# UCL-CCS/symmer

Measured on AMD Instinct MI355X. Metric: pauli_term_pairs_per_sec, higher is better.
Workload: dtype u64

## Files before the change

include/symgpu.h:

```cpp
#ifndef SYMGPU_H
#define SYMGPU_H
#include <stdint.h>

#ifdef __cplusplus
extern "C" {
#endif

#define SYMGPU_OK 0
#define SYMGPU_E_INVALID (-1)
#define SYMGPU_E_HIP (-2)
#define SYMGPU_E_NOMEM (-3)
#define SYMGPU_E_CAPACITY (-4)
#define SYMGPU_E_NODEVICE (-5)
#define SYMGPU_E_COLLISION (-6)
#define SYMGPU_E_RCCL (-7)

typedef struct symgpu_op_s *symgpu_op_t;

#define SYMGPU_MAX_DEVICES 16
int symgpu_init(int device);
int symgpu_init_all(int n_devices);
int symgpu_set_device(int device);
int symgpu_current_device(int *device);
int symgpu_n_initialised(int *n);
int symgpu_shutdown(void);
const char *symgpu_last_error(void);
int symgpu_device_count(int *n);
int symgpu_sync(void);
int symgpu_device_sync(void);
int symgpu_device_name(char *buf, int len);
int symgpu_mem_info(int64_t *free_bytes, int64_t *total_bytes);
int symgpu_timer_start(void);
int symgpu_timer_stop(float *ms);
#define SYMGPU_PROF_CLASSES 6
int symgpu_prof_enable(int kernel_class, int on);
int symgpu_prof_read(int kernel_class, int64_t *n_launches, double *total_ms);
#define SYMGPU_COUNTER_LIST(X) \
    X(HASH_RESEEDS, 0, "number of row-hash collisions that forced the cleanup to reseed its hash and retry (the exactness guard behind " \
      "symplectic_cleanup, operators/utils.py:230-279; expected 0 outside the tests, which weaken the hash on purpose)") \
    X(RESIDENT_DONE, 1, "rotations completed by the one-launch LDS-resident kernel") \
    X(RESIDENT_FAILED, 2, "calls of that kernel that reported a failed row verification or a barrier time-out (the multi-launch path then " \
      "recomputes)") \
    X(DEV_MALLOC_CALLS, 3, "device allocations that were not served from the allocator's arena") \
    X(RESIDENT_NS_PREPARE, 4, "host nanoseconds spent by the one-launch rotation in preparation") \
    X(RESIDENT_NS_LAUNCH, 5, "host nanoseconds spent by the one-launch rotation in the launch call") \
    X(RESIDENT_NS_WAIT, 6, "host nanoseconds spent by the one-launch rotation waiting for the kernel's status word") \
     \
    X(H2D_BYTES, 7, "payload bytes copied host -> device by this library (operators, coefficients, index arrays, result matrices; not the " \
      "few-byte counts and flags a call reads back)") \
    X(D2H_BYTES, 8, "payload bytes copied device -> host by this library (as 7)") \
    X(OP_UPLOADS, 9, "operator uploads (calls that moved a whole operator or its coefficients)") \
    X(OP_DOWNLOADS, 10, "operator downloads (calls that moved a whole operator or its coefficients)") \
    X(CANARY_HITS, 11, "device blocks whose guard bytes were overwritten (tuning build, SYMGPU_ALLOC_CANARY)") \
    X(CTX_MAX_THREADS, 12, "the most threads seen using one device's context at once since load, counted where a call uses the context's " \
      "state, whichever lock it took (1 while the per-device lock holds)") \
    X(CTX_WAITS, 13, "calls that found their device busy with another thread's call and waited") \
    X(CTX_UNLOCKED_USES, 14, "uses of a device's context by a call that did not hold that context's lock (0 while the lock is taken on the " \
      "right device)") \
     \
    X(GF2_BLOCKS_PANELLED, 15, "blocks (of up to 64 rows) panelled by the blocked GF(2) elimination since load - the one-workgroup path for " \
      "matrices of at most 64 rows and 64 words counts none") \
    X(GF2_PANEL_FULL_ROWS, 16, "of 15, the blocks whose panel ran on the full rows in LDS") \
    X(GF2_PANEL_WINDOW, 17, "of 15, the blocks whose panel ran on the two-word window (the rest took the four-word window, or held zero " \
      "rows only)") \
     \
    X(COMMUTE_REGISTER_TILE, 18, "commutation calls (symgpu_commutes, symgpu_commutes_dev, symgpu_commutes_bits_dev and what is built on " \
      "them) served by the register-tile kernel") \
    X(COMMUTE_WIDE_ROWS, 19, "commutation calls served by the wide-row kernel") \
    X(COMMUTE_M4R_TILE, 20, "launches of the Four-Russians commutation kernel with one tile per workgroup (a stream-K request with fewer " \
      "tiles than compute units counts here)") \
    X(COMMUTE_M4R_STREAMK, 21, "launches of the Four-Russians commutation kernel as stream-K (persistent workgroups over the (tile, step) " \
      "space)") \
     \
    X(CHAIN_REGISTERS, 22, "runs of Clifford rotations (symgpu_rotate_clifford_chain_dev with at least one row and one rotation, and the " \
      "runs that symgpu_perform_rotations_dev hands to it) served by the register chain") \
    X(CHAIN_LDS, 23, "runs of Clifford rotations served by the LDS-resident kernel") \
    X(CHAIN_SINGLE_WORKGROUP, 24, "runs of Clifford rotations served by the single-workgroup kernel") \
    X(CHAIN_TWO_LAUNCHES, 25, "runs of Clifford rotations served by the two-launch form") \
    X(CHAIN_FOUR_LAUNCHES, 26, "runs of Clifford rotations served by the four-launch form") \
    X(CHAIN_SORT_ONE_LAUNCH, 27, "segments (of up to 40 rotations) of the register chain whose keys were sorted by the one-launch sort (a " \
      "run that is redone after a time-out of the one-launch sort counts 27 and 28)") \
    X(CHAIN_SORT_LAUNCHES, 28, "segments (of up to 40 rotations) of the register chain whose keys were sorted by the multi-launch sort") \
    X(ROTATE_HASH_JOIN, 29, "single rotations (symgpu_rotate_single_dev) completed by the hash join") \
    X(ROTATE_CLIFFORD_FAST, 30, "single rotations completed by the Clifford fast path") \
    X(ROTATE_GENERAL, 31, "single rotations completed by the general path (stack + cleanup)") \
    X(ROTATE_GENERAL_BY_DUP_CHECK, 32, "of 31, odd-k Clifford rotations whose duplicate check found two equal rows") \
     \
    X(RESIDENT_LDS, 33, "one-launch rotations LAUNCHED (completed or not) with each block's rows in LDS") \
    X(RESIDENT_REGISTERS, 34, "one-launch rotations LAUNCHED (completed or not) with each block's rows in LDS and registers") \
    X(RESIDENT_ROWS_IN_MEMORY, 35, "one-launch rotations LAUNCHED (completed or not) with each block's rows left in memory") \
     \
    X(FLOW_COMPLETE_SORT, 36, "the packed pair keys were ordered by the complete sort, no flag pass") \
    X(FLOW_FLAGS_HASH_TABLES, 37, "the flag pass was launched from the bucketed operand hash tables") \
    X(FLOW_FLAGS_PARTIAL_SORT, 38, "the flag pass was launched behind the partial sort") \
    X(FLOW_FLAGS_GAVE_UP, 39, "a flag pass came back with its give-up word set") \
    X(GIVEUP_PRODUCT_BUCKET, 40, "of 39, the hash-table pass by reason (one each for every reason it reported): a product bucket of more " \
      "than 16,384 pairs") \
    X(GIVEUP_COUNTER_SATURATED, 41, "of 39, the hash-table pass by reason: a saturated 4-bit counter") \
    X(GIVEUP_LIST_OVERFLOW, 42, "of 39, the hash-table pass by reason: an overflowing list") \
    X(GIVEUP_OPERAND_BUCKET, 43, "of 39, the hash-table pass by reason: an operand bucket of more than 255 terms") \
    X(FLOW_SORTED_WHOLE, 44, "the sort was finished on the whole array after the flag pass (most keys flagged, a give-up, or " \
      "SYMGPU_CLEANUP_SUSPECTS=2)") \
    X(FLOW_SORTED_FLAGGED, 45, "the flagged keys were sorted alone") \
    X(FLOW_MARKED_FROM_BYTES, 46, "the single terms were marked from one byte per pair") \
    X(FLOW_FULL_SORT_REPEAT, 47, "the attempt was repeated with the full 64-bit sort (a long run of equal key prefixes that holds " \
      "different keys)") \
     \
    X(PRODUCT_ROWS_ONLY, 48, "all-pairs products by path: rows only") \
    X(PRODUCT_PHASE_STREAM, 49, "all-pairs products by path: phase-byte row stream") \
    X(PRODUCT_WIDE_COEFF_THEN_ROWS, 50, "all-pairs products by path: wide coefficient kernel, then rows") \
    X(PRODUCT_WORD_MAJOR_THEN_ROWS, 51, "all-pairs products by path: word-major coefficient kernel, then rows") \
    X(PRODUCT_WORD_MAJOR_BESIDE_ROWS, 52, "all-pairs products by path: the same beside the rows on a second stream") \
     \
    X(CSR_FILL_LDS, 53, "launches of the fill kernel of symgpu_to_csr_fill (k_csr_fill) with its slots in LDS") \
    X(CSR_FILL_SCRATCH, 54, "launches of the fill kernel of symgpu_to_csr_fill (k_csr_fill) with its slots in global scratch") \
     \
    X(DEV_BLOCKS_LIVE, 55, "a GAUGE, not a count: device blocks handed out by the allocator and not yet returned to it (operators, their " \
      "caches, scratch, what the contexts keep); never below 0") \
    X(DEV_FREE_UNKNOWN, 56, "blocks returned to the allocator that it did not hold (a double free, a pointer from elsewhere); the call " \
      "fails with SYMGPU_E_INVALID and nothing is released") \
     \
    X(OP_WORD_MAJOR_BUILDS, 57, "word-major copies of an operator's rows built into its handle (op_wordmajor, layout.hip)") \
    X(OP_BIT_MAJOR_BUILDS, 58, "bit-major copies of an operator's rows built into its handle for the Four-Russians commutation kernel " \
      "(m4r_bit_major, commute_m4r.hip; a copy built into the call's scratch counts nothing)") \
    X(OP_YCOUNT_BUILDS, 59, "Y-count arrays built into an operator's handle (op_ycount, layout.hip)") \
    X(OP_ROW_HASH_BUILDS, 60, "row-hash arrays computed from an operand's rows into its handle (analyze_rows, rotate_analyze.hip; " \
      "ensure_row_hashes, rotate_resident.hip); hashes a rotation hands on to its result count nothing")
#define SYMGPU_COUNTER_ENUM_ENTRY(name, id, text) SYMGPU_CTR_##name = id,
typedef enum symgpu_counter { SYMGPU_COUNTER_LIST(SYMGPU_COUNTER_ENUM_ENTRY) SYMGPU_CTR_COUNT = 61 } symgpu_counter;
#undef SYMGPU_COUNTER_ENUM_ENTRY
int symgpu_debug_counter(int which, int64_t *value);
const char *symgpu_debug_counter_name(int which);
int symgpu_debug_sort(uint64_t *keys, uint32_t *vals, int64_t n, int begin_bit, int end_bit, int form, int with_first_hist, int *form_ran);
int symgpu_debug_scan(const uint32_t *in, uint32_t *out, int64_t n, uint32_t *total);
int symgpu_debug_popc_scan(const uint64_t *bits, int64_t n_words, int64_t n32, uint32_t *out, uint32_t *total);
int symgpu_degraded(char *buf, int len);
int symgpu_debug_rotation_trace(uint64_t *out, int max_workgroups, int *n_workgroups);

int symgpu_membw_probe(int64_t bytes, double *fill_GBps, double *copy_GBps);

int symgpu_op_upload(const uint64_t *rows, const double *coeff , int64_t T, int Wq, symgpu_op_t *out);
int symgpu_op_alloc(int64_t capacity_rows, int Wq, int with_coeff, symgpu_op_t *out);
int symgpu_op_download(symgpu_op_t op, uint64_t *rows, double *coeff , int64_t capacity_rows);
int symgpu_op_info(symgpu_op_t op, int64_t *T, int *Wq, int64_t *capacity_rows);
int symgpu_op_free(symgpu_op_t op);
int symgpu_op_set_rows(symgpu_op_t op, int64_t T);
int symgpu_op_write(symgpu_op_t op, int64_t row_offset, const uint64_t *rows, const double *coeff , int64_t count);
int symgpu_op_copy_rows(symgpu_op_t dst, int64_t dst_offset, symgpu_op_t src, int64_t src_offset, int64_t count);
int symgpu_op_random(int64_t T, int n_qubits, double density, uint64_t seed, symgpu_op_t *out);
int symgpu_op_clone(symgpu_op_t in, symgpu_op_t *out);
int symgpu_op_set_coeff(symgpu_op_t op, const double *coeff_host);
int symgpu_op_scale(symgpu_op_t op, double re, double im, int conjugate_first);
int symgpu_op_ycount(symgpu_op_t op, int64_t *out_host);
int symgpu_op_upload_bool(const uint8_t *symp , const double *coeff , int64_t T, int n_qubits, symgpu_op_t *out);
int symgpu_op_download_bool(symgpu_op_t op, int n_qubits, uint8_t *symp_out , int64_t capacity_rows);
int symgpu_op_checksum(symgpu_op_t op, uint64_t *xor_words , double *coeff_sum );
int symgpu_op_popcount(symgpu_op_t op, uint64_t *sum);

int symgpu_ycount(const uint64_t *rows, int64_t T, int Wq, int64_t *out);

int symgpu_commutes(const uint64_t *A, int64_t N, const uint64_t *B, int64_t M, int Wq, uint8_t *out);
int symgpu_commutes_dev(symgpu_op_t A, int64_t a_begin, int64_t a_end, symgpu_op_t B, uint8_t *out_dev);
int symgpu_commutes_bits_dev(symgpu_op_t A, int64_t a_begin, int64_t a_end, symgpu_op_t B, uint64_t *out_bits_dev);
int symgpu_dev_alloc(int64_t bytes, void **ptr);
int symgpu_dev_free(void *ptr);
int symgpu_dev_download(const void *dev, void *host, int64_t bytes);
int symgpu_dev_upload(void *dev, const void *host, int64_t bytes);
int symgpu_dev_checksum_u8(const uint8_t *dev, int64_t n, uint64_t *sum);
int symgpu_dev_popcount_u64(const uint64_t *dev, int64_t n_words, uint64_t *sum);

int symgpu_mul_allpairs(const uint64_t *inner, const double *ci, int64_t Ni,
                        const uint64_t *outer, const double *co, int64_t No, int Wq, int inner_is_left,
                        uint64_t *out_rows, double *out_coeff);
int symgpu_mul_allpairs_dev(symgpu_op_t inner, symgpu_op_t outer, int64_t o_begin, int64_t o_end,
                            int inner_is_left, symgpu_op_t out);

int symgpu_cleanup(const uint64_t *rows, const double *coeff, int64_t T, int W, double thr, int use_thr,
                   uint64_t *out_rows, double *out_coeff, int64_t capacity, int64_t *n_out);
int symgpu_cleanup_dev(symgpu_op_t in, double thr, int use_thr, symgpu_op_t *out);
int symgpu_mul_cleanup(const uint64_t *inner, const double *ci, int64_t Ni,
                       const uint64_t *outer, const double *co, int64_t No, int Wq, int inner_is_left,
                       double thr, int use_thr,
                       uint64_t *out_rows, double *out_coeff, int64_t capacity, int64_t *n_out);
int symgpu_mul_cleanup_dev(symgpu_op_t inner, symgpu_op_t outer, int inner_is_left, double thr, int use_thr,
                           symgpu_op_t *out);
int symgpu_cleanup_indexed_dev(symgpu_op_t in, double thr, int use_thr, symgpu_op_t *out);
int symgpu_mul_cleanup_indexed_dev(symgpu_op_t inner, symgpu_op_t outer, int inner_is_left, double thr, int use_thr, symgpu_op_t *out);
int symgpu_op_first_index(symgpu_op_t op, uint64_t *first_host, int64_t capacity_rows);
int symgpu_op_gather(symgpu_op_t op, const int64_t *idx_host, int64_t n, symgpu_op_t *out);
int symgpu_part_global_index(symgpu_op_t part, const int64_t *inner_idx_host, int64_t n_inner, const int64_t *outer_idx_host, int64_t n_outer,
                             int64_t Ni_global);
int symgpu_op_set_first_index(symgpu_op_t op, const uint64_t *first_host);
int symgpu_merge_indexed_dev(const symgpu_op_t *parts, int n_parts, int key_bits, int do_cleanup, double thr, int use_thr, symgpu_op_t *out);

int symgpu_rotate_single(const uint64_t *rows, const double *coeff, int64_t N, int Wq, const uint64_t *q_row,
                         double cos_t, double sin_t, int clifford_k, double thr,
                         uint64_t *out_rows, double *out_coeff, int64_t capacity, int64_t *n_out, int *all_commute);
int symgpu_rotate_single_dev(symgpu_op_t in, const uint64_t *q_row_host, double cos_t, double sin_t, int clifford_k,
                             double thr, symgpu_op_t *out, int *all_commute);
int symgpu_rotate_single_dev_n(symgpu_op_t in, const uint64_t *q_row_host, double cos_t, double sin_t, int clifford_k,
                               double thr, symgpu_op_t *out, int *all_commute, int64_t *n_out);

int symgpu_rotate_clifford_chain_dev(symgpu_op_t in, const uint64_t *q_rows_host, const int *ks_host, int64_t K, symgpu_op_t *out);
int symgpu_perform_rotations_dev(symgpu_op_t in, const uint64_t *q_rows_host, const double *cos_t, const double *sin_t, const int *ks_host, int64_t K,
                                 double thr, int clean, symgpu_op_t *out, uint8_t *acted, int64_t *n_done, int *clean_out);

int symgpu_rref(uint64_t *rows, int64_t R, int64_t Wc, int64_t *xor_count, int64_t *pivots);
int symgpu_rref_dev(uint64_t *rows_dev, int64_t R, int64_t Wc, int64_t *xor_count, int64_t *pivots_host);

int symgpu_symmetry_kernel(const uint64_t *H, int64_t M, int n_qubits, int Wq,
                           uint64_t *out, int64_t capacity, int64_t *k, int64_t *xor_count);
int symgpu_symmetry_kernel_dev(symgpu_op_t H, int n_qubits, uint64_t *out, int64_t capacity, int64_t *k,
                               int64_t *xor_count);

int symgpu_op_gf2_rank(symgpu_op_t op, int64_t *rank);
int symgpu_generators_dev(symgpu_op_t op, symgpu_op_t *out);
int symgpu_generator_reconstruction_dev(symgpu_op_t G, symgpu_op_t M, int n_qubits, int64_t *recon_host, uint8_t *mask_host);

int symgpu_project_dev(symgpu_op_t op, const uint64_t *stab_rows, int k, const uint64_t *neg_mask, const int *keep_qubits, int n_keep,
                       int n_qubits, double thr, int use_thr, symgpu_op_t *out, int64_t *n_survived );
int symgpu_noncontextual_dev(symgpu_op_t op, int *is_noncontextual);
int symgpu_state_inner_dev(symgpu_op_t a, symgpu_op_t b, double *out);

#define SYMGPU_EXPVAL_LDS 1
#define SYMGPU_EXPVAL_GLOBAL 2
int symgpu_expval_terms_dev(symgpu_op_t op, symgpu_op_t phi, symgpu_op_t psi, double *out_terms , double *out_total ,
                            int *form );

typedef struct symgpu_csr_s *symgpu_csr_t;
int symgpu_to_csr_count(symgpu_op_t op, int n_qubits, int64_t *nnz, int64_t *fill_scratch_bytes, symgpu_csr_t *plan);
int symgpu_to_csr_fill(symgpu_csr_t plan, double *data, void *indices, void *indptr, int index_bytes);

#define SYMGPU_MATVEC_DIRECT 1
struct symgpu_matvec_s;
int symgpu_matvec_plan(symgpu_op_t op, int n_qubits, struct symgpu_matvec_s **plan);
int symgpu_matvec_free(struct symgpu_matvec_s *plan);
int symgpu_matvec_info(struct symgpu_matvec_s *plan, int *n_qubits, int64_t *n_terms, int64_t *n_groups, int64_t *device_bytes);
int symgpu_matvec_apply(struct symgpu_matvec_s *plan, const double *x_dev, double *y_dev, int *form );
int symgpu_matvec_sector_mask(struct symgpu_matvec_s *plan_N, int64_t n_particles, uint8_t *keep_dev, int64_t *n_kept);
int symgpu_lanczos_step(struct symgpu_matvec_s *plan, const uint8_t *keep_dev , double *basis_dev, int64_t capacity, int64_t j,
                        double *alpha, double *beta);
int symgpu_vec_combine(const double *basis_dev, int64_t m, int n_qubits, const double *s_host, double *out_dev, int normalise);

#define SYMGPU_PAULI_ONE_PASS 1
#define SYMGPU_PAULI_TWO_PASS 2
int symgpu_from_matrix_dense(const double *matrix, int n_qubits, const uint64_t *basis_x, const uint64_t *basis_z, int64_t K, symgpu_op_t *out,
                             int64_t *n_out, double *coeff_out, int *form);
int symgpu_from_matrix_csr(const double *data, const void *indices, const void *indptr, int index_bytes, int64_t nnz, int n_qubits,
                           const uint64_t *basis_x, const uint64_t *basis_z, int64_t K, symgpu_op_t *out, int64_t *n_out, double *coeff_out, int *form);

#define SYMGPU_REL_C 0
#define SYMGPU_REL_AC 1
#define SYMGPU_REL_QWC 2
#define SYMGPU_CLIQUE_PAIRS 1
#define SYMGPU_CLIQUE_UNIONS 2
int symgpu_qwc_dev(symgpu_op_t A, int64_t a_begin, int64_t a_end, symgpu_op_t B, uint8_t *out_dev);
int symgpu_relation_degrees_dev(symgpu_op_t op, int relation, int64_t *deg_host );
int symgpu_clique_colour_dev(symgpu_op_t op, int relation, const int64_t *order_host ,
                             int32_t *colour_host , int64_t *n_colours, int64_t *info );

int symgpu_noncon_signs_dev(symgpu_op_t terms, symgpu_op_t gens, const uint64_t *sel , int sel_words, int8_t *signs );
int symgpu_noncon_search(const double *coeff, const uint64_t *mask, const int32_t *clique, int64_t T, int n_free, int64_t n_cliques,
                         double *best_energy, uint64_t *best_mask, double *energies , int64_t *info );

#define SYMGPU_UNIQUE_ID_BYTES 128
int symgpu_comm_available(void);
int symgpu_comm_unique_id(uint8_t id[SYMGPU_UNIQUE_ID_BYTES]);
int symgpu_comm_init(const uint8_t id[SYMGPU_UNIQUE_ID_BYTES], int rank, int nranks);
int symgpu_comm_destroy(void);
int symgpu_comm_abandon(void);
int symgpu_comm_allgather_op(symgpu_op_t shard, symgpu_op_t full);
int symgpu_comm_barrier(void);
int symgpu_comm_init_all(int n_devices);
int symgpu_comm_allgather_ops(const symgpu_op_t *shards, const symgpu_op_t *fulls, int n);

#ifdef __cplusplus
}
#endif
#endif
```

symmer_amd/_lib.py:

```python
import ctypes
import os

_HERE = os.path.dirname(os.path.abspath(__file__))
LIB_PATH = os.path.join(_HERE, 'libsymgpu.so')

OK, E_INVALID, E_HIP, E_NOMEM, E_CAPACITY, E_NODEVICE, E_COLLISION, E_RCCL = 0, -1, -2, -3, -4, -5, -6, -7
_NAMES = {E_INVALID: 'SYMGPU_E_INVALID', E_HIP: 'SYMGPU_E_HIP', E_NOMEM: 'SYMGPU_E_NOMEM',
          E_CAPACITY: 'SYMGPU_E_CAPACITY', E_NODEVICE: 'SYMGPU_E_NODEVICE', E_COLLISION: 'SYMGPU_E_COLLISION',
          E_RCCL: 'SYMGPU_E_RCCL'}


class SymgpuError(RuntimeError):
    def __init__(self, code, text):
        super().__init__(f'{_NAMES.get(code, code)}: {text}')
        self.code = code


c_i64, c_int, c_dbl, c_u64 = ctypes.c_int64, ctypes.c_int, ctypes.c_double, ctypes.c_uint64
P = ctypes.c_void_p
PP = ctypes.POINTER(ctypes.c_void_p)

SIGNATURES = {
    'symgpu_init': [c_int],
    'symgpu_shutdown': [],
    'symgpu_init_all': [c_int],
    'symgpu_set_device': [c_int],
    'symgpu_current_device': [P],
    'symgpu_n_initialised': [P],
    'symgpu_device_count': [P],
    'symgpu_sync': [],
    'symgpu_device_sync': [],
    'symgpu_device_name': [P, c_int],
    'symgpu_mem_info': [P, P],
    'symgpu_timer_start': [],
    'symgpu_timer_stop': [P],
    'symgpu_prof_enable': [c_int, c_int],
    'symgpu_prof_read': [c_int, P, P],
    'symgpu_debug_counter': [c_int, P],
    'symgpu_debug_counter_name': [c_int],
    'symgpu_debug_sort': [P, P, c_i64, c_int, c_int, c_int, c_int, P],
    'symgpu_debug_scan': [P, P, c_i64, P],
    'symgpu_debug_popc_scan': [P, c_i64, c_i64, P, P],
    'symgpu_debug_rotation_trace': [P, c_int, P],
    'symgpu_degraded': [P, c_int],
    'symgpu_membw_probe': [c_i64, P, P],
    'symgpu_op_upload': [P, P, c_i64, c_int, PP],
    'symgpu_op_alloc': [c_i64, c_int, c_int, PP],
    'symgpu_op_download': [P, P, P, c_i64],
    'symgpu_op_info': [P, P, P, P],
    'symgpu_op_free': [P],
    'symgpu_op_set_rows': [P, c_i64],
    'symgpu_op_write': [P, c_i64, P, P, c_i64],
    'symgpu_op_random': [c_i64, c_int, c_dbl, c_u64, PP],
    'symgpu_op_checksum': [P, P, P],
    'symgpu_op_clone': [P, PP],
    'symgpu_op_set_coeff': [P, P],
    'symgpu_op_scale': [P, c_dbl, c_dbl, c_int],
    'symgpu_op_ycount': [P, P],
    'symgpu_op_upload_bool': [P, P, c_i64, c_int, PP],
    'symgpu_op_download_bool': [P, c_int, P, c_i64],
    'symgpu_ycount': [P, c_i64, c_int, P],
    'symgpu_commutes': [P, c_i64, P, c_i64, c_int, P],
    'symgpu_commutes_dev': [P, c_i64, c_i64, P, P],
    'symgpu_commutes_bits_dev': [P, c_i64, c_i64, P, P],
    'symgpu_dev_alloc': [c_i64, PP],
    'symgpu_dev_free': [P],
    'symgpu_dev_download': [P, P, c_i64],
    'symgpu_dev_upload': [P, P, c_i64],
    'symgpu_dev_checksum_u8': [P, c_i64, P],
    'symgpu_dev_popcount_u64': [P, c_i64, P],
    'symgpu_op_popcount': [P, P],
    'symgpu_op_copy_rows': [P, c_i64, P, c_i64, c_i64],
    'symgpu_mul_allpairs': [P, P, c_i64, P, P, c_i64, c_int, c_int, P, P],
    'symgpu_mul_allpairs_dev': [P, P, c_i64, c_i64, c_int, P],
    'symgpu_cleanup': [P, P, c_i64, c_int, c_dbl, c_int, P, P, c_i64, P],
    'symgpu_cleanup_dev': [P, c_dbl, c_int, PP],
    'symgpu_mul_cleanup': [P, P, c_i64, P, P, c_i64, c_int, c_int, c_dbl, c_int, P, P, c_i64, P],
    'symgpu_mul_cleanup_dev': [P, P, c_int, c_dbl, c_int, PP],
    'symgpu_cleanup_indexed_dev': [P, c_dbl, c_int, PP],
    'symgpu_mul_cleanup_indexed_dev': [P, P, c_int, c_dbl, c_int, PP],
    'symgpu_op_first_index': [P, P, c_i64],
    'symgpu_op_gather': [P, P, c_i64, PP],
    'symgpu_part_global_index': [P, P, c_i64, P, c_i64, c_i64],
    'symgpu_op_set_first_index': [P, P],
    'symgpu_merge_indexed_dev': [P, c_int, c_int, c_int, c_dbl, c_int, PP],
    'symgpu_rotate_single': [P, P, c_i64, c_int, P, c_dbl, c_dbl, c_int, c_dbl, P, P, c_i64, P, P],
    'symgpu_rotate_single_dev': [P, P, c_dbl, c_dbl, c_int, c_dbl, PP, P],
    'symgpu_rotate_single_dev_n': [P, P, c_dbl, c_dbl, c_int, c_dbl, PP, P, P],
    'symgpu_rotate_clifford_chain_dev': [P, P, P, c_i64, PP],
    'symgpu_perform_rotations_dev': [P, P, P, P, P, c_i64, c_dbl, c_int, PP, P, P, P],
    'symgpu_rref': [P, c_i64, c_i64, P, P],
    'symgpu_rref_dev': [P, c_i64, c_i64, P, P],
    'symgpu_symmetry_kernel': [P, c_i64, c_int, c_int, P, c_i64, P, P],
    'symgpu_symmetry_kernel_dev': [P, c_int, P, c_i64, P, P],
    'symgpu_op_gf2_rank': [P, P],
    'symgpu_generators_dev': [P, PP],
    'symgpu_generator_reconstruction_dev': [P, P, c_int, P, P],
    'symgpu_project_dev': [P, P, c_int, P, P, c_int, c_int, c_dbl, c_int, PP, P],
    'symgpu_noncontextual_dev': [P, P],
    'symgpu_state_inner_dev': [P, P, P],
    'symgpu_expval_terms_dev': [P, P, P, P, P, P],
    'symgpu_qwc_dev': [P, c_i64, c_i64, P, P],
    'symgpu_relation_degrees_dev': [P, c_int, P],
    'symgpu_clique_colour_dev': [P, c_int, P, P, P, P],
    'symgpu_noncon_signs_dev': [P, P, P, c_int, P],
    'symgpu_noncon_search': [P, P, P, c_i64, c_int, c_i64, P, P, P, P],
    'symgpu_to_csr_count': [P, c_int, P, P, PP],
    'symgpu_to_csr_fill': [P, P, P, P, c_int],
    'symgpu_from_matrix_dense': [P, c_int, P, P, c_i64, PP, P, P, P],
    'symgpu_from_matrix_csr': [P, P, P, c_int, c_i64, c_int, P, P, c_i64, PP, P, P, P],
    'symgpu_matvec_plan': [P, c_int, PP],
    'symgpu_matvec_free': [P],
    'symgpu_matvec_info': [P, P, P, P, P],
    'symgpu_matvec_apply': [P, P, P, P],
    'symgpu_matvec_sector_mask': [P, c_i64, P, P],
    'symgpu_lanczos_step': [P, P, P, c_i64, c_i64, P, P],
    'symgpu_vec_combine': [P, c_i64, c_int, P, P, c_int],
    'symgpu_comm_available': [],
    'symgpu_comm_unique_id': [P],
    'symgpu_comm_init': [P, c_int, c_int],
    'symgpu_comm_destroy': [],
    'symgpu_comm_abandon': [],
    'symgpu_comm_allgather_op': [P, P],
    'symgpu_comm_barrier': [],
    'symgpu_comm_init_all': [c_int],
    'symgpu_comm_allgather_ops': [P, P, c_int],
}

_lib = None
_initialised_device = None


def load():
    global _lib
    if _lib is not None:
        return _lib
    if not os.path.exists(LIB_PATH):
        raise SymgpuError(E_NODEVICE, f'{LIB_PATH} not found — build it with `python -c "import __graft_entry__ as g; g.build()"` '
                                      f'or `make -C symmer_amd/csrc` (there is no CPU fallback)')
    lib = ctypes.CDLL(LIB_PATH, mode=os.RTLD_NOW | os.RTLD_LOCAL | getattr(os, 'RTLD_DEEPBIND', 0))
    for name, argtypes in SIGNATURES.items():
        fn = getattr(lib, name)
        fn.argtypes = argtypes
        fn.restype = c_int
    lib.symgpu_last_error.restype = ctypes.c_char_p
    lib.symgpu_last_error.argtypes = []
    lib.symgpu_debug_counter_name.restype = ctypes.c_char_p
    _lib = lib
    return lib


_counter_ids = None


def counter_ids():
    global _counter_ids
    if _counter_ids is None:
        name_of, ids, which = load().symgpu_debug_counter_name, {}, 0
        while name_of(which) is not None:
            ids[name_of(which).decode('ascii')] = which
            which += 1
        _counter_ids = ids
    return _counter_ids


def last_error():
    return load().symgpu_last_error().decode('utf-8', 'replace')


def check(rc):
    if rc != OK:
        raise SymgpuError(rc, last_error())


def degraded():
    buf = ctypes.create_string_buffer(2048)
    check(load().symgpu_degraded(ctypes.addressof(buf), 2048))
    text = buf.value.decode('utf-8', 'replace')
    return [t for t in text.split('; ') if t]


def device_count():
    n = c_int(0)
    check(load().symgpu_device_count(ctypes.addressof(n)))
    return n.value


def init(device=None):
    global _initialised_device
    lib = load()
    if device is None:
        if _initialised_device is not None:
            return _initialised_device
        device = int(os.environ.get('SYMGPU_DEVICE', os.environ.get('LOCAL_RANK', '0')))
    if _initialised_device == device:
        return device
    n = device_count()
    if n <= 0:
        raise SymgpuError(E_NODEVICE, 'no HIP device visible: the symplectic hot path needs an MI355X (no CPU fallback)')
    check(lib.symgpu_init(device % n))
    _initialised_device = device % n
    return _initialised_device


def set_device(device):
    check(load().symgpu_set_device(int(device)))


def current_device():
    d = c_int(-1)
    check(load().symgpu_current_device(ctypes.addressof(d)))
    return d.value


def lib():
    if _initialised_device is None:
        init()
    return _lib


def addr(a):
    return None if a is None else a.ctypes.data
```

symmer_amd/csrc/cleanup.hip:

```cpp
#include "cleanup_common.h"
#include <stdlib.h>

namespace symgpu {

__global__ void k_popc_words(const u32 *__restrict__ bits, i64 n_words, u32 *__restrict__ counts) {
    for (i64 w = (i64)blockIdx.x * blockDim.x + threadIdx.x; w < n_words; w += (i64)gridDim.x * blockDim.x) counts[w] = (u32)__popc(bits[w]);
}

static i64 emit_batch_words() {
    const i64 w = [] { const char *e = SG_TUNE("SYMGPU_EMIT_BATCH"); const int l = e ? atoi(e) : 17; return (i64)1 << (l >= 6 && l <= 26 ? l : 17); }();
    return w;
}
template <bool PAIR, bool TRI>
__global__ __launch_bounds__(256) void k_emit_meta(const u32 *__restrict__ markbits, const u32 *__restrict__ wordprefix, i64 w_begin, i64 w_end,
                                                    const double *__restrict__ sum_of, int wpw, u32 Ni,
                                                    uint2 *__restrict__ meta, double *__restrict__ out_coeff, LazyEmit lz, u64 *__restrict__ out_first) {
    __shared__ unsigned short s_list[4][2048];
    const int lane = threadIdx.x & 63, wave = threadIdx.x >> 6;
    unsigned short *list = s_list[wave];
    const u32 P0 = wordprefix[w_begin];
    const i64 n_chunks = (w_end - w_begin + wpw - 1) / wpw;
    for (i64 chunk = (i64)blockIdx.x * 4 + wave; chunk < n_chunks; chunk += (i64)gridDim.x * 4) {
        const i64 w = w_begin + chunk * wpw + lane;
        const u32 bits = (lane < wpw && w < w_end) ? markbits[w] : 0u;
        const u32 cnt = (u32)__popc(bits);
        u32 incl = cnt;
#pragma unroll
        for (int off = 1; off < 64; off <<= 1) {
            const u32 v = __shfl_up(incl, off);
            if (lane >= off) incl += v;
        }
        const u32 K = __shfl(incl, 63);
        if (K == 0) continue;
        const u32 p_base = __shfl(wordprefix[w_begin + chunk * wpw], 0);
        {
            u32 b = bits, k = incl - cnt;
            while (b) { list[k++] = (unsigned short)(lane * 32 + __builtin_ctz(b)); b &= b - 1; }
        }
        __builtin_amdgcn_fence(__ATOMIC_RELEASE, "wavefront");
        __builtin_amdgcn_wave_barrier();
        const u32 t_base = (u32)((w_begin + chunk * wpw) * 32);
        for (u32 k = lane; k < K; k += 64) {
            const u32 t = t_base + list[k];
            u32 ti = t, to = 0;
            if (PAIR && TRI) tri_pair(t, Ni, to, ti);
            else if (PAIR) { to = t / Ni; ti = t - to * Ni; }
            double2 cf;
            if (lz.mode == 0 || ((lz.patchbits[t >> 5] >> (t & 31u)) & 1u)) cf = reinterpret_cast<const double2 *>(sum_of)[t];
            else if (lz.mode == 1) {
                const int e = (int)(((lz.e_lo[t >> 5] >> (t & 31u)) & 1u) | (((lz.e_hi[t >> 5] >> (t & 31u)) & 1u) << 1));
                double cx, cy;
                pair_coefficient(lz.ci[2 * ti], lz.ci[2 * ti + 1], lz.co[2 * to], lz.co[2 * to + 1], e, cx, cy);
                if (lz.squared && ti != to) {
                    if (e & 1) { cx = 0.0; cy = 0.0; }
                    else { cx = __dadd_rn(cx, cx); cy = __dadd_rn(cy, cy); }
                }
                cf.x = __dadd_rn(0.0, cx); cf.y = __dadd_rn(0.0, cy);
            } else {
                const double2 c0 = reinterpret_cast<const double2 *>(lz.coeff)[t];
                cf.x = __dadd_rn(0.0, c0.x); cf.y = __dadd_rn(0.0, c0.y);
            }
            reinterpret_cast<double2 *>(out_coeff)[(i64)p_base + k] = cf;
            meta[(p_base - P0) + k] = make_uint2(ti, to);
            if (out_first) out_first[(i64)p_base + k] = PAIR ? (((u64)to << 32) | ti) : (u64)t;
        }
        __builtin_amdgcn_wave_barrier();
    }
}

template <bool PAIR, int RC>
__global__ __launch_bounds__(256) void k_emit_stream(const uint2 *__restrict__ meta, const u32 *__restrict__ p_begin, const u32 *__restrict__ p_end,
                                                      int Wq, int wsh, const u32x4 *__restrict__ rows, const u32x4 *__restrict__ inner,
                                                      const u32x4 *__restrict__ outer, u32x4 *__restrict__ out_rows) {
    const i64 P0 = *p_begin;
    const i64 n_chunks16 = ((i64)*p_end - P0) * Wq;
    const i64 b0 = (i64)blockIdx.x * (256 * RC);
    if (b0 >= n_chunks16) return;
    const i64 f0 = b0 + threadIdx.x;
    const i64 last = n_chunks16 - 1;
    uint2 m[RC];
    int c[RC];
#pragma unroll
    for (int k = 0; k < RC; ++k) {
        const i64 f = f0 + 256 * k < last ? f0 + 256 * k : last;
        const i64 slot = wsh >= 0 ? f >> wsh : f / Wq;
        c[k] = (int)(f - slot * Wq);
        m[k] = meta[slot];
    }
    u32x4 v[RC];
#pragma unroll
    for (int k = 0; k < RC; ++k)
        v[k] = PAIR ? (inner[(i64)m[k].x * Wq + c[k]] ^ outer[(i64)m[k].y * Wq + c[k]]) : rows[(i64)m[k].x * Wq + c[k]];
    u32x4 *dst = out_rows + P0 * Wq + f0;
    if (b0 + 256 * RC <= n_chunks16) {
#pragma unroll
        for (int k = 0; k < RC; ++k) __builtin_nontemporal_store(v[k], dst + 256 * k);
    } else {
#pragma unroll
        for (int k = 0; k < RC; ++k)
            if (f0 + 256 * k < n_chunks16) __builtin_nontemporal_store(v[k], dst + 256 * k);
    }
}

template <bool PAIR, bool TRI, int NW, int U>
__global__ __launch_bounds__(256) void k_emit_fused(const u64 *__restrict__ markbits64, const u32 *__restrict__ wordprefix, i64 T, const double *__restrict__ sum_of,
                                                     u32 Ni, int Wq, int wsh, const u32x4 *__restrict__ rows, const u32x4 *__restrict__ inner,
                                                     const u32x4 *__restrict__ outer, u32x4 *__restrict__ out_rows, double *__restrict__ out_coeff, LazyEmit lz,
                                                     u64 *__restrict__ out_first, int pfx_shift ,
                                                     int interleaved) {
    __shared__ u32 s_i[4][64 * NW], s_o[4][64 * NW];
    const int lane = threadIdx.x & 63, wave = threadIdx.x >> 6;
    const i64 per_xcd = ((i64)gridDim.x + 7) / 8;
    const i64 blk = interleaved ? (i64)blockIdx.x : (i64)(blockIdx.x & 7) * per_xcd + (blockIdx.x >> 3);
    const i64 w0 = (blk * 4 + wave) * NW;
    if (w0 * 64 >= T) return;
    u64 bits[NW];
    u32 off[NW + 1];
    off[0] = 0;
#pragma unroll
    for (int u = 0; u < NW; ++u) {
        const i64 w = w0 + u;
        bits[u] = w * 64 < T ? markbits64[w] : 0ULL;
        if (w * 64 < T && T - w * 64 < 64) bits[u] &= (1ULL << (T - w * 64)) - 1ULL;
        off[u + 1] = off[u] + (u32)__popcll(bits[u]);
    }
    const u32 K = off[NW];
    if (K == 0) return;
    const i64 p_base = wordprefix[w0 << pfx_shift];
    u32 o_min = 0xFFFFFFFFu, o_max = 0u;
    u32 ti_[NW], to_[NW], pw_[NW], el_[NW], eh_[NW];
    double2 ca_[NW], cb_[NW], cs_[NW];
    u32 o_first = 0, i_first = 0;
    if (PAIR) {
        const u32 t0 = (u32)__builtin_amdgcn_readfirstlane((int)(u32)(w0 * 64));
        if (TRI) tri_pair(t0, Ni, o_first, i_first);
        else { o_first = t0 / Ni; i_first = t0 - o_first * Ni; }
        o_first = (u32)__builtin_amdgcn_readfirstlane((int)o_first); i_first = (u32)__builtin_amdgcn_readfirstlane((int)i_first);
    }
#pragma unroll
    for (int u = 0; u < NW; ++u) {
        const i64 tt = (w0 + u) * 64 + lane;
        const u32 t = (u32)(tt < T ? tt : T - 1);
        ti_[u] = t; to_[u] = 0;
        if (PAIR) {
            u32 o = o_first;
            u64 i = (u64)i_first + (t - (u32)(w0 * 64));
            while (i >= Ni) { i -= Ni; ++o; if (TRI) i += o; }
            to_[u] = o; ti_[u] = (u32)i;
        }
        pw_[u] = lz.mode != 0 ? lz.patchbits[t >> 5] : 0xFFFFFFFFu;
        if (lz.mode == 1) {
            el_[u] = lz.e_lo[t >> 5]; eh_[u] = lz.e_hi[t >> 5];
            ca_[u] = reinterpret_cast<const double2 *>(lz.ci)[ti_[u]];
            cb_[u] = reinterpret_cast<const double2 *>(lz.co)[to_[u]];
        } else if (lz.mode == 2) {
            cs_[u] = reinterpret_cast<const double2 *>(lz.coeff)[t];
        }
    }
#pragma unroll
    for (int u = 0; u < NW; ++u) {
        if ((bits[u] >> lane) & 1ULL) {
            const u32 rank = off[u] + (u32)__popcll(bits[u] & ((1ULL << lane) - 1ULL));
            const u32 t = (u32)((w0 + u) * 64 + lane);
            const u32 ti = ti_[u], to = to_[u];
            double2 cf;
            if (lz.mode == 0 || ((pw_[u] >> (t & 31u)) & 1u)) cf = reinterpret_cast<const double2 *>(sum_of)[t];
            else if (lz.mode == 1) {
                const int e = (int)(((el_[u] >> (t & 31u)) & 1u) | (((eh_[u] >> (t & 31u)) & 1u) << 1));
                double cx, cy;
                pair_coefficient(ca_[u].x, ca_[u].y, cb_[u].x, cb_[u].y, e, cx, cy);
                if (lz.squared && ti != to) {
                    if (e & 1) { cx = 0.0; cy = 0.0; }
                    else { cx = __dadd_rn(cx, cx); cy = __dadd_rn(cy, cy); }
                }
                cf.x = __dadd_rn(0.0, cx); cf.y = __dadd_rn(0.0, cy);
            } else {
                cf.x = __dadd_rn(0.0, cs_[u].x); cf.y = __dadd_rn(0.0, cs_[u].y);
            }
            reinterpret_cast<double2 *>(out_coeff)[p_base + rank] = cf;
            if (out_first) out_first[p_base + rank] = PAIR ? (((u64)to << 32) | ti) : (u64)t;
            s_i[wave][rank] = ti; s_o[wave][rank] = to;
            o_min = to < o_min ? to : o_min; o_max = to > o_max ? to : o_max;
        }
    }
    __builtin_amdgcn_fence(__ATOMIC_RELEASE, "wavefront");
    __builtin_amdgcn_wave_barrier();
    __builtin_amdgcn_fence(__ATOMIC_ACQUIRE, "wavefront");
    const u32 n_ch = K * (u32)Wq;
    u32x4 *dst = out_rows + p_base * Wq;
    bool one_outer = false;
    if (PAIR && wsh >= 0 && Wq <= 64 && lz.no_one_outer == 0) {
#pragma unroll
        for (int sft = 32; sft > 0; sft >>= 1) {
            const u32 a = (u32)__shfl_xor((int)o_min, sft), b = (u32)__shfl_xor((int)o_max, sft);
            o_min = a < o_min ? a : o_min; o_max = b > o_max ? b : o_max;
        }
        one_outer = o_min == o_max;
    }
    if (one_outer) {
        const u32x4 oc = outer[(i64)o_min * Wq + (lane & (Wq - 1))];
        for (u32 f0 = 0; f0 < n_ch; f0 += 64 * U) {
            u32x4 v[U];
#pragma unroll
            for (int u = 0; u < U; ++u) {
                const u32 f = f0 + 64 * u + lane < n_ch ? f0 + 64 * u + lane : n_ch - 1;
                const u32 r = f >> wsh;
                v[u] = inner[(i64)s_i[wave][r] * Wq + (lane & (Wq - 1))] ^ oc;
            }
#pragma unroll
            for (int u = 0; u < U; ++u)
                if (f0 + 64 * u + lane < n_ch) __builtin_nontemporal_store(v[u], dst + f0 + 64 * u + lane);
        }
        return;
    }
    for (u32 f0 = 0; f0 < n_ch; f0 += 64 * U) {
        u32x4 v[U];
#pragma unroll
        for (int u = 0; u < U; ++u) {
            const u32 f = f0 + 64 * u + lane < n_ch ? f0 + 64 * u + lane : n_ch - 1;
            const u32 r = wsh >= 0 ? f >> wsh : f / (u32)Wq;
            const u32 c = f - r * (u32)Wq;
            v[u] = PAIR ? (inner[(i64)s_i[wave][r] * Wq + c] ^ outer[(i64)s_o[wave][r] * Wq + c]) : rows[(i64)s_i[wave][r] * Wq + c];
        }
#pragma unroll
        for (int u = 0; u < U; ++u)
            if (f0 + 64 * u + lane < n_ch) __builtin_nontemporal_store(v[u], dst + f0 + 64 * u + lane);
    }
}

struct TouchMaps { const u32x4 *p[5]; i64 n16[5]; };
__global__ __launch_bounds__(256) void k_touch(TouchMaps tm, u32 *__restrict__ sink) {
    u32 acc = 0;
#pragma unroll
    for (int m = 0; m < 5; ++m)
        for (i64 i = (i64)blockIdx.x * 256 + threadIdx.x; i < tm.n16[m]; i += (i64)gridDim.x * 256) { const u32x4 v = tm.p[m][i]; acc |= v.x & v.y & v.z & v.w; }
    if (acc == 0xDEADBEEFu) *sink = acc;
}

__global__ void k_popc_words64_tail(const u64 *__restrict__ bits, i64 n64, i64 n32, u32 *__restrict__ counts) {
    for (i64 w = (i64)blockIdx.x * blockDim.x + threadIdx.x; w < n64; w += (i64)gridDim.x * blockDim.x) {
        u64 b = bits[w];
        if (w == n64 - 1 && (n32 & 1)) b &= 0xFFFFFFFFULL;
        counts[w] = (u32)__popcll(b);
    }
}
int emit_prefix(const u32 *markbits_p, i64 T, Scratch &wordprefix, Scratch &total, bool wide) {
    hipStream_t st = ctx().stream;
    const i64 n_words = (T + 31) / 32, n64 = (T + 63) / 64;
    const i64 n = wide ? n64 : n_words;
    SG_TRY(wordprefix.alloc((size_t)n * 4));
    SG_TRY(total.alloc(32));
    if (wide && n64 <= POPC_SCAN_SMALL_MAX) return popc_scan_small(reinterpret_cast<const u64 *>(markbits_p), n64, n_words, wordprefix.as<u32>(), total.as<u32>());
    if (wide) hipLaunchKernelGGL(k_popc_words64_tail, dim3(grid_for(n64)), dim3(256), 0, st, reinterpret_cast<const u64 *>(markbits_p), n64, n_words, wordprefix.as<u32>());
    else hipLaunchKernelGGL(k_popc_words, dim3(grid_for(n_words)), dim3(256), 0, st, markbits_p, n_words, wordprefix.as<u32>());
    KERNEL_CHECK();
    return exclusive_scan_u32(wordprefix.as<u32>(), wordprefix.as<u32>(), n, total.as<u32>());
}

struct EmitOrder { int interleaved = 0; EmitProbe *probe = nullptr; };
static int emit_order_begin(const void *dst, size_t bytes, EmitOrder &eo) {
    Context &c = ctx();
    if (const char *e = getenv("SYMGPU_EMIT_ORDER")) { eo.interleaved = e[0] == '1'; return SYMGPU_OK; }
    if (bytes < ((size_t)512 << 20)) return SYMGPU_OK;
    EmitProbe *p = nullptr, *oldest = &c.emit_probe[0];
    for (auto &q : c.emit_probe) {
        if (q.key == dst) { p = &q; break; }
        if (q.stamp < oldest->stamp) oldest = &q;
    }
    if (!p) { p = oldest; p->key = dst; p->phase = 0; p->best[0] = p->best[1] = 1e30f; }
    p->stamp = ++c.emit_stamp;
    if (p->phase > 0 && p->phase <= 4) {
        float ms = 0;
        if (hipEventSynchronize(p->ev[1]) == hipSuccess && hipEventElapsedTime(&ms, p->ev[0], p->ev[1]) == hipSuccess) {
            const int o = (p->phase - 1) & 1;
            if (ms < p->best[o]) p->best[o] = ms;
        } else (void)hipGetLastError();
        if (p->phase == 4) { p->choice = p->best[1] < p->best[0] ? 1 : 0; p->phase = 5; }
    }
    if (p->phase >= 5) { eo.interleaved = p->choice; return SYMGPU_OK; }
    if (!p->ev[0]) { HIP_TRY(hipEventCreate(&p->ev[0])); HIP_TRY(hipEventCreate(&p->ev[1])); }
    eo.interleaved = p->phase & 1;
    eo.probe = p;
    HIP_TRY(hipEventRecord(p->ev[0], c.stream));
    return SYMGPU_OK;
}
static void emit_order_end(const EmitOrder &eo) {
    if (!eo.probe) return;
    (void)hipEventRecord(eo.probe->ev[1], ctx().stream);
    ++eo.probe->phase;
}

int emit_touch(const u32 *markbits_p, i64 T, const LazyEmit &lz, EmitPrefix &pre) {
    const i64 n16 = (T + 63) / 64 / 2;
    pre.touched = true;
    if (n16 <= 0 || T < ((i64)1 << 23)) return SYMGPU_OK;
    TouchMaps tm;
    const void *maps[5] = {markbits_p, pre.wordprefix.p, lz.mode ? (const void *)lz.patchbits : nullptr, lz.mode == 1 ? (const void *)lz.e_lo : nullptr,
                           lz.mode == 1 ? (const void *)lz.e_hi : nullptr};
    for (int m = 0; m < 5; ++m) {
        tm.p[m] = reinterpret_cast<const u32x4 *>(maps[m]);
        tm.n16[m] = maps[m] ? (m == 1 ? (pre.wide ? n16 / 2 : 2 * n16) : n16) : 0;
    }
    hipLaunchKernelGGL(k_touch, dim3(grid_for(2 * n16)), dim3(256), 0, ctx().stream, tm, pre.total.as<u32>() + 2);
    KERNEL_CHECK();
    return SYMGPU_OK;
}
int cleanup_finish(u32 *markbits_p, const double *sum_of_p, i64 T, bool pair, const u64 *rows, int W, const u64 *inner, i64 Ni,
                   const u64 *outer, symgpu_op_t *out, int Wq_out, bool tri, const LazyEmit &lz, bool want_first, const CleanupSwitches &sw,
                   EmitPrefix &pre) {
    hipStream_t st = ctx().stream;
    const i64 n_words = (T + 31) / 32;
    Scratch &wordprefix = pre.wordprefix, &total = pre.total;
    const i64 n_out = pre.n_out;
    OwnedOp res;
    SG_TRY(res.alloc(rows_or_one(n_out), n_out, Wq_out, true));
    if (want_first) SG_TRY(res.attach_first());
    if (n_out > 0) {
        const int Wq = W / 2;
        const int wsh = (Wq & (Wq - 1)) == 0 ? __builtin_ctz((unsigned)Wq) : -1;
        const u32x4 *pin = reinterpret_cast<const u32x4 *>(inner), *pout = reinterpret_cast<const u32x4 *>(outer);
        u32x4 *dst = reinterpret_cast<u32x4 *>(res->rows);
        const bool fused = sw.fused(Wq);
        if (fused) {
            const i64 n_w64 = (T + 63) / 64;
            const int shape = sw.emit_shape;
            const int NWs = shape / 16, Us = shape % 16;
            const int NWr = (NWs == 1 || NWs == 4 || NWs == 8) ? NWs : 2;
            const dim3 gfu((unsigned)(((n_w64 + 4 * NWr - 1) / (4 * NWr) + 7) / 8 * 8));
            if (sw.emit_touch != 0 && !pre.touched) SG_TRY(emit_touch(markbits_p, T, lz, pre));
            EmitOrder eo;
            SG_TRY(emit_order_begin(dst, (size_t)n_out * (size_t)(16 * Wq + 16), eo));
            ProfScope prof(3);
#define LAUNCH_FUSED_S(P, TR, NWV, UV) hipLaunchKernelGGL((k_emit_fused<P, TR, NWV, UV>), gfu, dim3(256), 0, st, reinterpret_cast<const u64 *>(markbits_p), wordprefix.as<u32>(), T, sum_of_p, \
                                               (u32)(pair ? Ni : 1), Wq, wsh, reinterpret_cast<const u32x4 *>(rows), pin, pout, dst, res->coeff, lz, res->first, pre.wide ? 0 : 1, eo.interleaved)
#define LAUNCH_FUSED_U(P, TR, NWV) do { if (Us == 8) LAUNCH_FUSED_S(P, TR, NWV, 8); else if (Us == 2) LAUNCH_FUSED_S(P, TR, NWV, 2); else LAUNCH_FUSED_S(P, TR, NWV, 4); } while (0)
#define LAUNCH_FUSED(P, TR) do { if (NWr == 1) LAUNCH_FUSED_U(P, TR, 1); else if (NWr == 4) LAUNCH_FUSED_U(P, TR, 4); else if (NWr == 8) LAUNCH_FUSED_U(P, TR, 8); \
                                 else LAUNCH_FUSED_U(P, TR, 2); } while (0)
            if (pair && tri) LAUNCH_FUSED(true, true); else if (pair) LAUNCH_FUSED(true, false); else LAUNCH_FUSED(false, false);
            emit_order_end(eo);
#undef LAUNCH_FUSED_S
#undef LAUNCH_FUSED_U
#undef LAUNCH_FUSED
        } else {
        const int rc_env = sw.emit_rc;
        const int RCs = rc_env == 1 || rc_env == 4 ? rc_env : 2;
        const i64 EMIT_BATCH_WORDS = emit_batch_words();
        const i64 bw = n_words < EMIT_BATCH_WORDS ? n_words : EMIT_BATCH_WORDS;
        Scratch meta;
        SG_TRY(meta.alloc((size_t)bw * 32 * sizeof(uint2)));
        int wpw = 64;
        while (wpw > 1 && (bw + wpw - 1) / wpw < 16384) wpw >>= 1;
        for (i64 w0 = 0; w0 < n_words; w0 += EMIT_BATCH_WORDS) {
            const i64 w1 = w0 + EMIT_BATCH_WORDS < n_words ? w0 + EMIT_BATCH_WORDS : n_words;
            i64 ge = ((w1 - w0 + wpw - 1) / wpw + 3) / 4;
            if (ge > 16384) ge = 16384;
#define LAUNCH_META(P, TR) hipLaunchKernelGGL((k_emit_meta<P, TR>), dim3((unsigned)ge), dim3(256), 0, st, markbits_p, wordprefix.as<u32>(), w0, w1, sum_of_p, wpw, \
                                              (u32)(pair ? Ni : 1), meta.as<uint2>(), res->coeff, lz, res->first)
            if (pair && tri) LAUNCH_META(true, true); else if (pair) LAUNCH_META(true, false); else LAUNCH_META(false, false);
#undef LAUNCH_META
            const u32 *p_begin = wordprefix.as<u32>() + w0;
            const u32 *p_end = w1 < n_words ? wordprefix.as<u32>() + w1 : total.as<u32>();
            const i64 gs = ((w1 - w0) * 32 * Wq + 256 * RCs - 1) / (256 * RCs);
#define LAUNCH_STREAM(P, R) hipLaunchKernelGGL((k_emit_stream<P, R>), dim3((unsigned)gs), dim3(256), 0, st, meta.as<uint2>(), p_begin, p_end, Wq, wsh, \
                                               reinterpret_cast<const u32x4 *>(rows), pin, pout, dst)
            {
                ProfScope prof(3);
                if (pair) { if (RCs == 1) LAUNCH_STREAM(true, 1); else if (RCs == 4) LAUNCH_STREAM(true, 4); else LAUNCH_STREAM(true, 2); }
                else { if (RCs == 1) LAUNCH_STREAM(false, 1); else if (RCs == 4) LAUNCH_STREAM(false, 4); else LAUNCH_STREAM(false, 2); }
            }
#undef LAUNCH_STREAM
        }
        }
        KERNEL_CHECK();
        HIP_TRY(hipStreamSynchronize(st));
    }
    res->dup_free = 1;
    res.hand_out(out);
    return SYMGPU_OK;
}

}
```

symmer_amd/csrc/cleanup_common.h:

```cpp
#pragma once
#include "common.h"
#include "sort.h"

namespace symgpu {

struct PackedLayout {
    int bi, bo;
    __host__ __device__ int F() const { return bi + bo + 2; }
    __device__ __forceinline__ u32 i(u64 k) const { return (u32)(k & ((1ULL << bi) - 1ULL)); }
    __device__ __forceinline__ u32 o(u64 k) const { return (u32)((k >> bi) & ((1ULL << bo) - 1ULL)); }
    __device__ __forceinline__ int e(u64 k) const { return (int)((k >> (bi + bo)) & 3ULL); }
    __device__ __forceinline__ u32 fields(u64 k) const { return (u32)(k & ((1ULL << (bi + bo)) - 1ULL)); }
    __device__ __forceinline__ u64 full_key(const u64 *__restrict__ hI, const u64 *__restrict__ hO, u64 k) const { return hI[i(k)] ^ hO[o(k)]; }
};
__device__ __forceinline__ u32 tri_slot(u32 o, u32 i, u32 N) { return (u32)((u64)o * N - (u64)o * (o - 1) / 2 - o + i); }
__device__ __forceinline__ void tri_pair(u32 p, u32 N, u32 &o, u32 &i) {
    const double b = 2.0 * N + 1.0;
    i64 oo = (i64)((b - sqrt(b * b - 8.0 * (double)p)) * 0.5);
    if (oo < 0) oo = 0;
    if (oo > (i64)N - 1) oo = (i64)N - 1;
    auto off = [&](i64 x) { return x * (i64)N - x * (x - 1) / 2; };
    while (oo > 0 && off(oo) > (i64)p) --oo;
    while (oo + 1 < (i64)N && off(oo + 1) <= (i64)p) ++oo;
    o = (u32)oo;
    i = (u32)((i64)p - off(oo) + oo);
}

constexpr int SUS_RUN_BITS = 16;

static int sorted_bits(i64 n, int cap) {
    int lg = 0;
    while (((i64)1 << lg) < n) ++lg;
    const int want = (lg + 5 + 7) / 8 * 8;
    return want < cap ? want : cap;
}

struct CleanupSwitches {
    bool unpacked = false;
    bool nosquare = false;
    int lazy = -1;
    int suspects = 1;
    bool key_bytes = true;
    bool nofloor = false;
    bool emit_fused = true;
    i64 hs_waves = (i64)1 << 21;
    bool zero_seg = true;
    int emit_touch = -1;
    bool emit_no_one_outer = false;
    int emit_shape = 2 * 16 + 4;
    int emit_rc = 2;
    bool fused(int Wq) const { return Wq <= 64 && emit_fused; }
};

struct CleanupRequest {
    bool pair = false;
    const u64 *rows = nullptr;
    const double *coeff = nullptr;
    PairOperands p;
    i64 T = 0;
    int W = 0, Wq_out = 0;
    double thr = 0.0;
    int use_thr = 0;
    bool want_first = false;
};

struct CleanupPlan {
    PackedLayout L{0, 0};
    bool packed = false;
    bool squared = false;
    i64 Tk = 0;
    int nbits = 64;
    bool lazy_call = false;
    bool lazy = false;
    bool sus_try = false;
    bool key_bytes = false;
};

struct LazyEmit {
    int mode = 0, squared = 0, no_one_outer = 0;
    const u32 *patchbits = nullptr, *e_lo = nullptr, *e_hi = nullptr;
    const double *ci = nullptr, *co = nullptr, *coeff = nullptr;
};
struct EmitPrefix { Scratch wordprefix, total; i64 n_out = -1; bool touched = false, wide = false; };


struct CleanupRun {
    CleanupRequest rq;
    CleanupSwitches sw;
    CleanupPlan pl;
    hipStream_t st = nullptr;
    bool same_rows = false;
    const u64 *hO_p = nullptr;
    const double *coeff = nullptr;
    u64 seed = 1;
    Scratch keys, keys2, idx, idx2, fixlist, collision, hI, hO, pair_coeff, markbits, sum_of, zpart, zcount, patchbits, e_lo, e_hi, dirtybits, sort_hist, cfloor;
    Scratch diag_seq;
    bool diag_side = false;
    EmitPrefix pre;
    struct Attempt {
        u32 *first_hist = nullptr;
        i64 Tsort = 0;
        int fix_bits = 64;
        bool sus_active = false, sus_coop = false;
        u64 *ks = nullptr;
        u32 *is = nullptr;
        bool mark_zeroed = false, merges_found = false, patch_zeroed = false;
        bool lazy = false;
        Attempt() {}
        explicit Attempt(const CleanupPlan &pl) : Tsort(pl.Tk), fix_bits(pl.nbits), lazy(pl.lazy) {}
    } a;
};

int hash_rows_any(const u64 *rows, i64 T, int W, u64 seed, u64 *out1, u32 *iota);
int cleanup_hash_keys(CleanupRun &r);
int cleanup_order(CleanupRun &r);
int zero_two(void *a, size_t bytes_a, void *b, size_t bytes_b, void *c = nullptr, size_t bytes_c = 0);
int cleanup_diag_begin(CleanupRun &r);
int cleanup_fixups(CleanupRun &r);
int cleanup_segment_sums(CleanupRun &r);
int emit_prefix(const u32 *markbits_p, i64 T, Scratch &wordprefix, Scratch &total, bool wide);
int emit_touch(const u32 *markbits_p, i64 T, const LazyEmit &lz, EmitPrefix &pre);
int cleanup_finish(u32 *markbits_p, const double *sum_of_p, i64 T, bool pair, const u64 *rows, int W, const u64 *inner, i64 Ni,
                   const u64 *outer, symgpu_op_t *out, int Wq_out, bool tri, const LazyEmit &lz, bool want_first, const CleanupSwitches &sw,
                   EmitPrefix &pre);

}
```

symmer_amd/csrc/cleanup_driver.hip:

```cpp
#include "cleanup_common.h"
#include <stdlib.h>
#include <stdio.h>

namespace symgpu {

static CleanupSwitches read_cleanup_switches() {
    CleanupSwitches sw;
    const char *e = nullptr;
    if ((e = getenv("SYMGPU_CLEANUP_UNPACKED"))) sw.unpacked = e[0] == '1';
    if ((e = getenv("SYMGPU_CLEANUP_NOSQUARE"))) sw.nosquare = e[0] == '1';
    if ((e = getenv("SYMGPU_CLEANUP_LAZY"))) sw.lazy = e[0] == '0' ? 0 : 1;
    if ((e = getenv("SYMGPU_CLEANUP_SUSPECTS"))) sw.suspects = e[0] == '0' ? 0 : e[0] == '2' ? 2 : 1;
    if ((e = getenv("SYMGPU_CLEANUP_KEYBYTES"))) sw.key_bytes = e[0] != '0';
    sw.nofloor = getenv("SYMGPU_CLEANUP_NOFLOOR") != nullptr;
    if ((e = getenv("SYMGPU_EMIT_FUSED"))) sw.emit_fused = e[0] != '0';
    if ((e = SG_TUNE("SYMGPU_HS_WAVES"))) sw.hs_waves = atoll(e);
    if ((e = SG_TUNE("SYMGPU_CLEANUP_ZEROSEG"))) sw.zero_seg = e[0] != '0';
    if ((e = SG_TUNE("SYMGPU_EMIT_TOUCH"))) sw.emit_touch = e[0] != '0';
    sw.emit_no_one_outer = SG_TUNE("SYMGPU_EMIT_NO_ONE_OUTER") != nullptr;
    if ((e = SG_TUNE("SYMGPU_EMIT_SHAPE"))) { int nw = 2, u = 4; sscanf(e, "%d,%d", &nw, &u); sw.emit_shape = nw * 16 + u; }
    if ((e = SG_TUNE("SYMGPU_EMIT_RC"))) sw.emit_rc = atoi(e);
    return sw;
}

static CleanupPlan plan_cleanup(const CleanupRequest &rq, const CleanupSwitches &sw, bool full_sort = false) {
    CleanupPlan pl;
    const PairOperands &p = rq.p;
    while (rq.pair && ((i64)1 << pl.L.bi) < p.Ni) ++pl.L.bi;
    while (rq.pair && ((i64)1 << pl.L.bo) < p.No) ++pl.L.bo;
    pl.packed = rq.pair && pl.L.bi + pl.L.bo <= 32 && pl.L.bi < 32 && !sw.unpacked && !full_sort;
    pl.squared = pl.packed && p.inner == p.outer && p.Ni == p.No && p.ci == p.co && rq.use_thr && rq.thr > 0.0 && !sw.nosquare;
    pl.Tk = pl.squared ? p.Ni * (p.Ni + 1) / 2 : rq.T;
    const int hash_bits = pl.packed ? 64 - pl.L.F() : 64;
    pl.nbits = full_sort ? 64 : sorted_bits(pl.Tk, hash_bits);
    pl.lazy_call = sw.lazy == 1 || (sw.lazy == -1 && rq.pair);
    pl.lazy = pl.lazy_call && (sw.lazy == 1 || pl.Tk >= ((i64)1 << (pl.squared ? 20 : 18)));
    pl.sus_try = pl.packed && pl.lazy && sw.suspects != 0 && pl.nbits == 32 && (pl.Tk >> SUS_RUN_BITS) <= 2048 && !(p.inner == p.outer && !pl.squared);
    pl.key_bytes = pl.sus_try && pair_dups_fits(p.Ni, p.No, pl.squared, pl.Tk, nullptr) && !wide_pairs_worthwhile(p.Ni, p.No, rq.W / 2) && sw.key_bytes;
    return pl;
}

static LazyEmit lazy_emit(const CleanupRun &r) {
    LazyEmit lz; lz.no_one_outer = r.sw.emit_no_one_outer ? 1 : 0;
    if (r.a.lazy) {
        lz.mode = r.pl.packed ? 1 : 2; lz.squared = r.pl.squared ? 1 : 0;
        lz.patchbits = r.patchbits.as<u32>(); lz.e_lo = r.e_lo.as<u32>(); lz.e_hi = r.e_hi.as<u32>();
        lz.ci = r.rq.p.ci; lz.co = r.rq.p.co; lz.coeff = r.coeff;
    }
    return lz;
}

static int cleanup_status(CleanupRun &r, u32 hback[4]) {
    EmitPrefix &pre = r.pre;
    pre.wide = r.sw.fused(r.rq.W / 2);
    SG_TRY(emit_prefix(r.markbits.as<u32>(), r.pl.Tk, pre.wordprefix, pre.total, pre.wide));
    pre.touched = false;
    if (pre.wide && r.sw.emit_touch == -1)
        SG_TRY(emit_touch(r.markbits.as<u32>(), r.pl.Tk, lazy_emit(r), pre));
    SG_TRY(read_back_words(pre.total.as<u32>(), 1, r.collision.as<u32>(), 2, hback, r.a.sus_coop ? radix_sort_coop_flag() : nullptr));
    pre.n_out = hback[0];
    return SYMGPU_OK;
}

static int cleanup_run(const CleanupRequest &rq, symgpu_op_t *out) {
    if (rq.T >= ((i64)1 << 32) - 1) {
        set_error("cleanup: %lld terms exceed the 2^32-2 limit of the 32-bit index sort", (long long)rq.T);
        return SYMGPU_E_INVALID;
    }
    if (rq.T == 0) {
        OwnedOp res;
        SG_TRY(res.alloc(1, 0, rq.Wq_out, true));
        res->dup_free = 1;
        res.hand_out(out);
        return SYMGPU_OK;
    }
    CleanupRun r;
    r.rq = rq; r.sw = read_cleanup_switches(); r.pl = plan_cleanup(rq, r.sw);
    r.st = ctx().stream; r.coeff = rq.coeff;
    r.same_rows = rq.pair && rq.p.outer == rq.p.inner && rq.p.No == rq.p.Ni;
    const i64 T = rq.T;
    const size_t bitmap_bytes = (size_t)((T + 63) / 64) * 8;
    SG_TRY(r.keys.alloc((size_t)T * 8));
    SG_TRY(r.keys2.alloc((size_t)T * 8));
    SG_TRY(r.markbits.alloc(bitmap_bytes));
    if (r.pl.lazy_call) {
        SG_TRY(r.patchbits.alloc(bitmap_bytes));
        if (rq.pair) { SG_TRY(r.e_lo.alloc(bitmap_bytes)); SG_TRY(r.e_hi.alloc(bitmap_bytes)); }
    }
    SG_TRY(r.sum_of.alloc((size_t)T * 16));
    SG_TRY(r.collision.alloc(16));
    if (rq.pair) {
        SG_TRY(r.hI.alloc((size_t)rq.p.Ni * 8));
        if (!r.same_rows) SG_TRY(r.hO.alloc((size_t)rq.p.No * 8));
        r.hO_p = r.same_rows ? r.hI.as<u64>() : r.hO.as<u64>();
    } else {
        SG_TRY(r.idx.alloc((size_t)T * 4));
        SG_TRY(r.idx2.alloc((size_t)T * 4));
    }
    r.seed = ctx().hash_tab ? ctx().hash_seed : 1;
    struct JoinSide {
        bool &pending;
        ~JoinSide() { if (pending) (void)hipStreamWaitEvent(ctx().stream, ctx().ev_join, 0); }
    } join_side{r.diag_side};
    if (r.pl.squared) SG_TRY(cleanup_diag_begin(r));
    bool ok = false;
    for (int attempt = 0; attempt < 6 && !ok; ++attempt) {
        r.a = CleanupRun::Attempt(r.pl);
        SG_TRY(ensure_hash_tables(r.seed));
        SG_TRY(cleanup_hash_keys(r));
        SG_TRY(cleanup_order(r));
        SG_TRY(cleanup_fixups(r));
        SG_TRY(cleanup_segment_sums(r));
        u32 hback[4] = {0, 0, 0, 0};
        SG_TRY(cleanup_status(r, hback));
        if (r.a.sus_coop) {
            bool timed_out = false;
            radix_sort_coop_note(hback[3], &timed_out);
            if (timed_out) continue;
        }
        if (hback[2]) { bump_counter(SYMGPU_CTR_FLOW_FULL_SORT_REPEAT); r.pl = plan_cleanup(rq, r.sw, true); continue; }
        ok = (hback[1] == 0);
        if (!ok) { ++r.seed; bump_counter(SYMGPU_CTR_HASH_RESEEDS); }
    }
    if (!ok) { set_error("cleanup: 64-bit row-hash collision survived 4 reseeds"); return SYMGPU_E_COLLISION; }
    const PairOperands &p = rq.p;
    return cleanup_finish(r.markbits.as<u32>(), r.sum_of.as<double>(), r.pl.Tk, rq.pair, rq.rows, rq.W, p.inner, p.Ni, p.outer, out, rq.Wq_out,
                          r.pl.squared, lazy_emit(r), rq.want_first, r.sw, r.pre);
}

int cleanup_rows(const u64 *rows, const double *coeff, i64 T, int W, double thr, int use_thr, symgpu_op_t *out, int Wq_out, bool want_first) {
    CleanupRequest rq;
    rq.rows = rows; rq.coeff = coeff; rq.T = T; rq.W = W; rq.Wq_out = Wq_out; rq.thr = thr; rq.use_thr = use_thr; rq.want_first = want_first;
    return cleanup_run(rq, out);
}

int cleanup_pairs(const PairOperands &p, double thr, int use_thr, symgpu_op_t *out, bool want_first) {
    CleanupRequest rq;
    rq.pair = true; rq.p = p; rq.T = p.Ni * p.No; rq.W = p.W; rq.Wq_out = p.Wq_out; rq.thr = thr; rq.use_thr = use_thr; rq.want_first = want_first;
    return cleanup_run(rq, out);
}

int finish_to_host(OwnedOp &res, const char *what, uint64_t *out_rows, double *out_coeff, int64_t capacity, int64_t *n_out) {
    if (n_out) *n_out = res->T;
    if (res->T > capacity) {
        set_error("%s %lld < %lld rows", what, (long long)capacity, (long long)res->T);
        return SYMGPU_E_CAPACITY;
    }
    if (res->T > 0) SG_TRY(symgpu_op_download(res.op, out_rows, out_coeff, capacity));
    return SYMGPU_OK;
}

}

using namespace symgpu;

static PairOperands product_operands(symgpu_op_t inner, symgpu_op_t outer, int inner_is_left) {
    PairOperands p;
    p.inner = inner->rows; p.outer = outer->rows; p.ci = inner->coeff; p.co = outer->coeff;
    p.Ni = inner->T; p.No = outer->T; p.W = 2 * inner->Wq; p.Wq_out = inner->Wq; p.inner_is_left = inner_is_left;
    return p;
}

extern "C" {

int symgpu_cleanup_dev(symgpu_op_t in, double thr, int use_thr, symgpu_op_t *out) {
    SG_ENTER(in);
    SG_REQUIRE(in && out, "cleanup_dev: null handle");
    SG_REQUIRE(in->coeff || in->T == 0, "cleanup_dev: operator has no coefficients");
    return cleanup_rows(in->rows, in->coeff, in->T, 2 * in->Wq, thr, use_thr, out, in->Wq);
}

int symgpu_mul_cleanup_dev(symgpu_op_t inner, symgpu_op_t outer, int inner_is_left, double thr, int use_thr, symgpu_op_t *out) {
    SG_ENTER(inner, outer);
    SG_REQUIRE(inner && outer && out, "mul_cleanup_dev: null handle");
    SG_REQUIRE(inner->Wq == outer->Wq, "mul_cleanup_dev: operands must share Wq");
    const i64 Ni = inner->T, No = outer->T;
    if (Ni * No == 0) return cleanup_rows(nullptr, nullptr, 0, 2 * inner->Wq, thr, use_thr, out, inner->Wq);
    SG_REQUIRE(inner->coeff && outer->coeff, "mul_cleanup_dev: operands have no coefficients");
    SG_REQUIRE(No == 0 || Ni < ((i64)1 << 32) / No, "mul_cleanup_dev: Ni*No must stay below 2^32 (tile the outer operand)");
    return cleanup_pairs(product_operands(inner, outer, inner_is_left), thr, use_thr, out);
}

int symgpu_cleanup_indexed_dev(symgpu_op_t in, double thr, int use_thr, symgpu_op_t *out) {
    SG_ENTER(in);
    SG_REQUIRE(in && out, "cleanup_indexed_dev: null handle");
    SG_REQUIRE(in->coeff || in->T == 0, "cleanup_indexed_dev: operator has no coefficients");
    return cleanup_rows(in->rows, in->coeff, in->T, 2 * in->Wq, thr, use_thr, out, in->Wq, true);
}

int symgpu_mul_cleanup_indexed_dev(symgpu_op_t inner, symgpu_op_t outer, int inner_is_left, double thr, int use_thr, symgpu_op_t *out) {
    SG_ENTER(inner, outer);
    SG_REQUIRE(inner && outer && out, "mul_cleanup_indexed_dev: null handle");
    SG_REQUIRE(inner->Wq == outer->Wq, "mul_cleanup_indexed_dev: operands must share Wq");
    const i64 Ni = inner->T, No = outer->T;
    if (Ni * No == 0) return cleanup_rows(nullptr, nullptr, 0, 2 * inner->Wq, thr, use_thr, out, inner->Wq, true);
    SG_REQUIRE(inner->coeff && outer->coeff, "mul_cleanup_indexed_dev: operands have no coefficients");
    SG_REQUIRE(Ni < ((i64)1 << 32) / No, "mul_cleanup_indexed_dev: Ni*No must stay below 2^32 (tile the outer operand)");
    return cleanup_pairs(product_operands(inner, outer, inner_is_left), thr, use_thr, out, true);
}

int symgpu_op_first_index(symgpu_op_t op, uint64_t *first_host, int64_t capacity) {
    SG_ENTER(op);
    SG_REQUIRE(op && (first_host || op->T == 0), "op_first_index: null argument");
    SG_REQUIRE(op->first || op->T == 0, "op_first_index: the operator does not come from an *_indexed cleanup");
    if (capacity < op->T) { set_error("op_first_index: capacity %lld < %lld rows", (long long)capacity, (long long)op->T); return SYMGPU_E_CAPACITY; }
    if (op->T > 0) {
        HIP_TRY(hipMemcpyAsync(first_host, op->first, (size_t)op->T * 8, hipMemcpyDeviceToHost, ctx().stream));
        count_d2h((size_t)op->T * 8);
        HIP_TRY(hipStreamSynchronize(ctx().stream));
    }
    return SYMGPU_OK;
}

int symgpu_cleanup(const uint64_t *rows, const double *coeff, int64_t T, int W, double thr, int use_thr, uint64_t *out_rows,
                   double *out_coeff, int64_t capacity, int64_t *n_out) {
    SG_ENTER();
    SG_REQUIRE(T >= 0 && W >= 2 && (W % 2) == 0 && capacity >= 0, "cleanup: sizes (W must be 2*Wq)");
    SG_REQUIRE(T == 0 || (rows && coeff), "cleanup: null input");
    OwnedOp in, res;
    SG_TRY(symgpu_op_upload(rows, coeff, T, W / 2, in.slot()));
    SG_TRY(cleanup_rows(in->rows, in->coeff, T, W, thr, use_thr, res.slot(), W / 2));
    in.reset();
    return finish_to_host(res, "output capacity", out_rows, out_coeff, capacity, n_out);
}

int symgpu_mul_cleanup(const uint64_t *inner, const double *ci, int64_t Ni, const uint64_t *outer, const double *co, int64_t No,
                       int Wq, int inner_is_left, double thr, int use_thr, uint64_t *out_rows, double *out_coeff, int64_t capacity,
                       int64_t *n_out) {
    SG_ENTER();
    SG_REQUIRE(Ni >= 0 && No >= 0 && Wq >= 1 && capacity >= 0, "mul_cleanup: sizes");
    if (Ni == 0 || No == 0) { if (n_out) *n_out = 0; return SYMGPU_OK; }
    SG_REQUIRE(inner && outer && ci && co, "mul_cleanup: null input");
    OwnedOp a, b, res;
    SG_TRY(symgpu_op_upload(inner, ci, Ni, Wq, a.slot()));
    SG_TRY(symgpu_op_upload(outer, co, No, Wq, b.slot()));
    SG_TRY(symgpu_mul_cleanup_dev(a.op, b.op, inner_is_left, thr, use_thr, res.slot()));
    a.reset(); b.reset();
    return finish_to_host(res, "output capacity", out_rows, out_coeff, capacity, n_out);
}

}
```

symmer_amd/csrc/cleanup_keys.hip:

```cpp
#include "cleanup_common.h"

namespace symgpu {

__global__ void k_pair_keys(const u64 *__restrict__ hI, i64 Ni, const u64 *__restrict__ hO, i64 T, u64 *__restrict__ keys, u32 *__restrict__ idx) {
    for (i64 t = (i64)blockIdx.x * blockDim.x + threadIdx.x; t < T; t += (i64)gridDim.x * blockDim.x) {
        const i64 o = t / Ni, i = t - o * Ni;
        keys[t] = hI[i] ^ hO[o];
        idx[t] = (u32)t;
    }
}

__global__ __launch_bounds__(1024) void k_coeff_floor(const double *__restrict__ c0, i64 n0, const double *__restrict__ c1, i64 n1,
                                                      unsigned long long *__restrict__ slot0, int one_block) {
    const double *__restrict__ c = blockIdx.y ? c1 : c0;
    const i64 n = blockIdx.y ? n1 : n0;
    unsigned long long *slot = slot0 + blockIdx.y;
    __shared__ unsigned long long s_min;
    if (one_block) { if (threadIdx.x == 0) s_min = ~0ULL; __syncthreads(); }
    double m = __builtin_inf();
    const i64 stride = (i64)gridDim.x * blockDim.x;
    for (i64 t0 = (i64)blockIdx.x * blockDim.x + threadIdx.x; t0 < n; t0 += 4 * stride) {
        double2 v[4];
#pragma unroll
        for (int k = 0; k < 4; ++k) { const i64 t = t0 + k * stride; v[k] = reinterpret_cast<const double2 *>(c)[t < n ? t : n - 1]; }
#pragma unroll
        for (int k = 0; k < 4; ++k) {
            const double a = fabs(v[k].x), b = fabs(v[k].y);
            const double mx = (a <= __DBL_MAX__ && b <= __DBL_MAX__) ? (a > b ? a : b) : 0.0;
            m = mx < m ? mx : m;
        }
    }
#pragma unroll
    for (int d = 32; d >= 1; d >>= 1) { const double o = __shfl_xor(m, d); m = o < m ? o : m; }
    if ((threadIdx.x & 63) == 0) atomicMin(one_block ? &s_min : slot, (unsigned long long)__double_as_longlong(m));
    if (one_block) { __syncthreads(); if (threadIdx.x == 0) *slot = s_min; }
}
__device__ __forceinline__ bool floors_clear(double fi, double fo, double thr) { return 0.5 * fi * fo > thr && fi * fo > 0x1p-1000; }
template <bool PACKED>
__global__ __launch_bounds__(256) void k_mark_singles(const u64 *__restrict__ keys, const double *__restrict__ coeff, i64 space, PackedLayout L,
                                                       const double *__restrict__ ci, const double *__restrict__ co, int squared, double thr, int use_thr,
                                                       u64 *__restrict__ markbits64, u64 *__restrict__ e_lo64, u64 *__restrict__ e_hi64,
                                                       u32 *__restrict__ hist, int hist_shift, i64 n_tiles, const double *__restrict__ floor_i,
                                                       const double *__restrict__ floor_o) {
    __shared__ u32 s_h[256];
    const int lane = threadIdx.x & 63, wave = threadIdx.x >> 6;
    const bool all_kept = PACKED && (!use_thr || (floor_i && floor_o && floors_clear(floor_i[0], floor_o[0], thr)));
    if (hist) { s_h[threadIdx.x] = 0; __syncthreads(); }
    const i64 tile_base = (i64)blockIdx.x * SORT_TILE;
#pragma unroll 1
    for (int step = 0; step < SORT_TILE / 1024; ++step) {
        const i64 g0 = tile_base + step * 1024 + wave * 256;
        if (g0 >= space) break;
        u64 k[4];
        double2 cf[4];
#pragma unroll
        for (int j = 0; j < 4; ++j) {
            const i64 sidx = g0 + 64 * j + lane;
            k[j] = 0ULL; cf[j].x = 0.0; cf[j].y = 0.0;
            if (sidx < space) {
                if (PACKED) k[j] = keys[sidx];
                else cf[j] = reinterpret_cast<const double2 *>(coeff)[sidx];
            }
        }
        double2 ca[4], cb[4];
        if (PACKED && !all_kept) {
#pragma unroll
            for (int j = 0; j < 4; ++j) {
                const u32 i = L.i(k[j]), o = L.o(k[j]);
                ca[j] = reinterpret_cast<const double2 *>(ci)[i];
                cb[j] = reinterpret_cast<const double2 *>(co)[o];
            }
        }
#pragma unroll
        for (int j = 0; j < 4; ++j) {
            const i64 sidx = g0 + 64 * j + lane;
            if (g0 + 64 * j >= space) break;
            const bool valid = sidx < space;
            double cx = cf[j].x, cy = cf[j].y;
            int e = 0;
            bool keep;
            if (PACKED && all_kept) {
                if (valid && hist) atomicAdd(&s_h[(u32)(k[j] >> hist_shift) & 255u], 1u);
                e = L.e(k[j]);
                keep = valid && !(use_thr && squared && (e & 1) && L.i(k[j]) != L.o(k[j]) && !(0.0 > thr));
            } else {
            if (PACKED && valid) {
                if (hist) atomicAdd(&s_h[(u32)(k[j] >> hist_shift) & 255u], 1u);
                const u32 i = L.i(k[j]), o = L.o(k[j]);
                e = L.e(k[j]);
                pair_coefficient(ca[j].x, ca[j].y, cb[j].x, cb[j].y, e, cx, cy);
                if (squared && i != o) {
                    if (e & 1) { cx = 0.0; cy = 0.0; }
                    else { cx = __dadd_rn(cx, cx); cy = __dadd_rn(cy, cy); }
                }
            }
            keep = valid && (!use_thr || above_thr(cx, cy, thr));
            }
            const u64 mk = __ballot(keep);
            const i64 chunk = (g0 + 64 * j) / 64;
            if (PACKED) {
                const u64 lo = __ballot(e & 1), hi = __ballot(e & 2);
                if (lane == 0) { markbits64[chunk] = mk; e_lo64[chunk] = lo; e_hi64[chunk] = hi; }
            } else if (lane == 0) markbits64[chunk] = mk;
        }
    }
    if (hist) {
        __syncthreads();
        hist[(i64)blockIdx.x * 256 + threadIdx.x] = s_h[threadIdx.x];
    }
}

__device__ __forceinline__ void pair_of_index(i64 pos, i64 Ni, int squared, i64 &i, i64 &o) {
    if (!squared) { o = pos / Ni; i = pos - o * Ni; return; }
    const double b = 2.0 * (double)Ni + 1.0;
    i64 oo = (i64)((b - sqrt(b * b - 8.0 * (double)pos)) * 0.5);
    if (oo < 0) oo = 0;
    if (oo >= Ni) oo = Ni - 1;
    while (oo > 0 && oo * (2 * Ni - oo + 1) / 2 > pos) --oo;
    while (oo + 1 < Ni && (oo + 1) * (2 * Ni - oo) / 2 <= pos) ++oo;
    o = oo;
    i = pos - oo * (2 * Ni - oo + 1) / 2 + oo;
}
__device__ __forceinline__ u32 pack_bit0_of_bytes(u32 w) { return ((w & 0x01010101u) * 0x01020408u) >> 24 & 0xFu; }
__global__ __launch_bounds__(256) void k_mark_bytes(const u32x4 *__restrict__ eb, i64 space, i64 n_groups, i64 Ni, const double *__restrict__ ci,
                                                     const double *__restrict__ co, int squared, double thr, int use_thr, unsigned short *__restrict__ mark16,
                                                     unsigned short *__restrict__ lo16, unsigned short *__restrict__ hi16, const double *__restrict__ floor_i,
                                                     const double *__restrict__ floor_o) {
    const bool all_kept = !use_thr || (floor_i && floor_o && floors_clear(floor_i[0], floor_o[0], thr));
    const bool drop_rule = use_thr && squared && !(0.0 > thr);
    for (i64 g = (i64)blockIdx.x * blockDim.x + threadIdx.x; g < n_groups; g += (i64)gridDim.x * blockDim.x) {
        const i64 p0 = g * 16;
        u32x4 v = {0u, 0u, 0u, 0u};
        if (p0 < space) v = __builtin_nontemporal_load(eb + g);
        u32 valid = 0xFFFFu;
        if (p0 + 16 > space) valid = p0 < space ? (1u << (int)(space - p0)) - 1u : 0u;
        u32 lo = 0, hi = 0, drop = 0;
#pragma unroll
        for (int q = 0; q < 4; ++q) {
            const u32 w = v[q];
            lo |= pack_bit0_of_bytes(w) << (4 * q);
            hi |= pack_bit0_of_bytes(w >> 1) << (4 * q);
            drop |= pack_bit0_of_bytes(w & ~(w >> 2)) << (4 * q);
        }
        lo &= valid; hi &= valid;
        u32 keep;
        if (all_kept) keep = valid & (drop_rule ? ~drop : 0xFFFFu);
        else {
            keep = 0;
            for (int k = 0; k < 16; ++k) {
                if (!((valid >> k) & 1u)) continue;
                i64 i, o;
                pair_of_index(p0 + k, Ni, squared, i, o);
                const int e = (int)(((lo >> k) & 1u) | (((hi >> k) & 1u) << 1));
                double cx, cy;
                pair_coefficient(ci[2 * i], ci[2 * i + 1], co[2 * o], co[2 * o + 1], e, cx, cy);
                if (squared && i != o) {
                    if (e & 1) { cx = 0.0; cy = 0.0; }
                    else { cx = __dadd_rn(cx, cx); cy = __dadd_rn(cy, cy); }
                }
                const bool kp = !use_thr || above_thr(cx, cy, thr);
                keep |= (kp ? 1u : 0u) << k;
            }
        }
        mark16[g] = (unsigned short)keep; lo16[g] = (unsigned short)lo; hi16[g] = (unsigned short)hi;
    }
}
__global__ __launch_bounds__(256) void k_keys_of_indices(u64 *__restrict__ out, const u32 *__restrict__ n_flagged, const unsigned char *__restrict__ eb, i64 Ni, int squared,
                                                          PackedLayout L, const u64 *__restrict__ hI, const u64 *__restrict__ hO) {
    const u64 hmask = ~((1ULL << L.F()) - 1ULL);
    const i64 n = n_flagged[0];
    for (i64 t = (i64)blockIdx.x * blockDim.x + threadIdx.x; t < n; t += (i64)gridDim.x * blockDim.x) {
        const i64 pos = (i64)out[t];
        i64 i, o;
        pair_of_index(pos, Ni, squared, i, o);
        const u64 e = eb[pos] & 3u;
        out[t] = ((hI[i] ^ hO[o]) & hmask) | (e << (L.bi + L.bo)) | ((u64)o << L.bi) | (u64)i;
    }
}

constexpr int SUS_TILE = 4096;
constexpr int SUS_BLOOM = 17;
constexpr int SUS_CAND = 960;
constexpr int SUS_MAX_EXT = 64;
constexpr int SUS_WAVES = 8;
constexpr int SUS_ROWS = SUS_TILE / (64 * SUS_WAVES), SUS_XROWS = 1024 / (64 * SUS_WAVES);
__device__ __forceinline__ u32 wave_shr1(u32 v, u32 lane0) {
    return (u32)__builtin_amdgcn_update_dpp((int)lane0, (int)v, 0x138, 0xf, 0xf, false);
}
__device__ __forceinline__ u32 sus_slot(u32 w) { return __builtin_amdgcn_alignbit(w, w, 16) & ((1u << SUS_BLOOM) - 1u); }
static_assert(SUS_BLOOM == 17 && SUS_RUN_BITS == 16, "sus_slot is written for these");
__global__ __launch_bounds__(64 * SUS_WAVES) __attribute__((amdgpu_waves_per_eu(8, 8))) void k_find_suspects(const u64 *__restrict__ keys, i64 T, PackedLayout L, const u64 *__restrict__ hI,
                                                                   const u64 *__restrict__ hO, u64 *__restrict__ suspect64, u32 *__restrict__ giveup) {
    constexpr int NT = 64 * SUS_WAVES;
    __shared__ u32 s_seen[1 << (SUS_BLOOM - 5)], s_dup[1 << (SUS_BLOOM - 5)];
    __shared__ __attribute__((aligned(16))) u32 s_cw[SUS_CAND];
    __shared__ u32 s_cpos[SUS_CAND];
    __shared__ u32 s_start, s_end[2], s_nc;
    const int lane = threadIdx.x & 63, wave = threadIdx.x >> 6;
    const u64 lt_mask = (1ULL << lane) - 1ULL;
    const i64 t0 = (i64)blockIdx.x * SUS_TILE;
    const u64 *kt = keys + t0;
    const u32 n_rel = T - t0 < (i64)0x0fffffff ? (u32)(T - t0) : 0x0fffffffu;
    const u32 t1_rel = n_rel < (u32)SUS_TILE ? n_rel : (u32)SUS_TILE;
    const u32 rmask = (1u << SUS_RUN_BITS) - 1u;
    const int F = L.F();
    typedef unsigned long long ull;
    auto at = [&](u32 rel) -> u64 { return *reinterpret_cast<const u64 *>(reinterpret_cast<const char *>(kt) + (size_t)((rel < n_rel ? rel : n_rel - 1) << 3)); };
    auto hash0 = [&](u64 k) -> bool { return (k >> F) == 0ULL; };
    constexpr int NK = SUS_ROWS + SUS_XROWS;
    u64 key[NK];
    const u32 wrel = (u32)wave * (64 * SUS_ROWS), xrel = (u32)SUS_TILE + (u32)wave * (64 * SUS_XROWS);
    auto rel_of = [&](int r) -> u32 { return (r < SUS_ROWS ? wrel + r * 64 : xrel + (r - SUS_ROWS) * 64) + lane; };
#pragma unroll
    for (int r = 0; r < NK; ++r) key[r] = at(rel_of(r));
    u32 w[NK], zmask = 0;
    const u64 kprev = wrel > 0 ? at(wrel - 1) : (t0 > 0 ? keys[t0 - 1] : 0ULL);
    const u64 kpe = at(xrel - 1);
    {
        const u32x4 z = {0u, 0u, 0u, 0u};
#pragma unroll
        for (int k = 0; k < (1 << (SUS_BLOOM - 5)) / (4 * NT); ++k) {
            reinterpret_cast<u32x4 *>(s_seen)[k * NT + threadIdx.x] = z;
            reinterpret_cast<u32x4 *>(s_dup)[k * NT + threadIdx.x] = z;
        }
    }
    if (threadIdx.x == 0) { s_start = ~0u; s_end[0] = ~0u; s_end[1] = ~0u; s_nc = 0u; }
    __syncthreads();
#pragma unroll
    for (int r = 0; r < NK; ++r) { w[r] = (u32)(key[r] >> 32); zmask |= (hash0(key[r]) ? 1u : 0u) << r; }
    {
        u32 carry = (u32)(kprev >> 32) & rmask;
        u32 first_b = ~0u, first_e = ~0u;
#pragma unroll
        for (int r = 0; r < NK; ++r) {
            if (r == SUS_ROWS) carry = (u32)(kpe >> 32) & rmask;
            const u32 v = w[r] & rmask;
            const u32 pv = wave_shr1(v, carry);
            carry = (u32)__builtin_amdgcn_readlane((int)v, 63);
            const u32 rel = rel_of(r);
            if (r < SUS_ROWS) {
                const u64 bm = __ballot(rel < t1_rel && (v != pv || (t0 == 0 && rel == 0)));
                if (bm && first_b == ~0u) first_b = rel - lane + (u32)__builtin_ctzll(bm);
            } else {
                const u64 bm = __ballot(rel < n_rel && v != pv);
                if (bm && first_e == ~0u) first_e = rel - lane + (u32)__builtin_ctzll(bm);
            }
        }
        if (lane == 0 && first_b != ~0u) atomicMin(&s_start, first_b);
        if (lane == 0 && first_e != ~0u) atomicMin(&s_end[0], first_e);
    }
    __syncthreads();
    const u32 s_rel = s_start;
    if (s_rel == ~0u) return;
    u32 e_rel = t1_rel;
    bool closed = n_rel <= (u32)SUS_TILE;
    if (!closed) {
        const u32 end_now = s_end[0];
        const u32 step_end = (u32)SUS_TILE + 1024u;
        if (end_now != ~0u) { e_rel = end_now; closed = true; }
        else if (step_end >= n_rel) { e_rel = n_rel; closed = true; }
        else e_rel = step_end;
    }
    auto flag_chunk = [&](u64 m, i64 chunk) {
        if (lane == 0 && m) atomicOr(reinterpret_cast<ull *>(suspect64 + chunk), (ull)m);
    };
    {
        u32 ins = 0;
#pragma unroll
        for (int r = 0; r < NK; ++r) {
            const u32 rel = rel_of(r);
            const bool own = rel >= s_rel && rel < e_rel;
            const bool zh = own && ((zmask >> r) & 1u);
            flag_chunk(__ballot(zh), (t0 + rel - lane) / 64);
            ins |= ((own && !zh) ? 1u : 0u) << r;
        }
#pragma unroll
        for (int h = 0; h < 2; ++h) {
            constexpr int HB = NK / 2;
            u32 old[HB];
#pragma unroll
            for (int q = 0; q < HB; ++q) {
                const int r = h * HB + q;
                const u32 slot = sus_slot(w[r]), in = (ins >> r) & 1u;
                old[q] = atomicOr(&s_seen[slot >> 5], in << (slot & 31));
            }
#pragma unroll
            for (int q = 0; q < HB; ++q) {
                const int r = h * HB + q;
                const u32 slot = sus_slot(w[r]), in = (ins >> r) & 1u;
                atomicOr(&s_dup[slot >> 5], old[q] & (in << (slot & 31)));
            }
        }
    }
    for (int step = 1; !closed; ++step) {
        if (step == SUS_MAX_EXT) {
            if (threadIdx.x == 0) atomicOr(giveup, 1u);
            return;
        }
        const u32 q0 = xrel + (u32)step * 1024u;
        u64 kq[SUS_XROWS];
#pragma unroll
        for (int r = 0; r < SUS_XROWS; ++r) kq[r] = at(q0 + r * 64 + lane);
        const u64 kp = at(q0 - 1);
        u32 carry = (u32)(kp >> 32) & rmask, first_e = ~0u;
#pragma unroll
        for (int r = 0; r < SUS_XROWS; ++r) {
            const u32 rel = q0 + r * 64 + lane;
            const u32 v = (u32)(kq[r] >> 32) & rmask;
            const u32 pv = wave_shr1(v, carry);
            carry = (u32)__builtin_amdgcn_readlane((int)v, 63);
            const u64 bm = __ballot(rel < n_rel && v != pv);
            if (bm && first_e == ~0u) first_e = q0 + r * 64 + (u32)__builtin_ctzll(bm);
        }
        if (lane == 0 && first_e != ~0u) atomicMin(&s_end[step & 1], first_e);
        __syncthreads();
        const u32 end_now = s_end[step & 1];
        const u32 step_end = (u32)SUS_TILE + (u32)(step + 1) * 1024u;
        if (end_now != ~0u) { e_rel = end_now; closed = true; }
        else if (step_end >= n_rel) { e_rel = n_rel; closed = true; }
        else e_rel = step_end;
#pragma unroll
        for (int r = 0; r < SUS_XROWS; ++r) {
            const u32 rel = q0 + r * 64 + lane;
            const bool own = rel < e_rel;
            const bool zh = own && hash0(kq[r]);
            flag_chunk(__ballot(zh), (t0 + q0) / 64 + r);
            const u32 wq = (u32)(kq[r] >> 32), slot = sus_slot(wq);
            const u32 bit = (own && !zh) ? 1u << (slot & 31) : 0u;
            const u32 old = atomicOr(&s_seen[slot >> 5], bit);
            atomicOr(&s_dup[slot >> 5], old & bit);
        }
    }
    __syncthreads();
    auto listed = [&](u32 rel, u32 wk, bool zh) -> bool {
        const u32 slot = sus_slot(wk);
        return rel >= s_rel && rel < e_rel && ((s_dup[slot >> 5] >> (slot & 31)) & 1u) && !zh;
    };
    {
        u64 m[NK];
        u32 total = 0;
#pragma unroll
        for (int r = 0; r < NK; ++r) {
            m[r] = __ballot(listed(rel_of(r), w[r], (zmask >> r) & 1u));
            total += (u32)__popcll(m[r]);
        }
        if (total) {
            u32 base = 0;
            if (lane == 0) base = atomicAdd(&s_nc, total);
            base = (u32)__builtin_amdgcn_readfirstlane((int)base);
#pragma unroll
            for (int r = 0; r < NK; ++r) {
                const u32 n = base + (u32)__popcll(m[r] & lt_mask);
                if (((m[r] >> lane) & 1ULL) && n < (u32)SUS_CAND) { s_cpos[n] = rel_of(r); s_cw[n] = w[r]; }
                base += (u32)__popcll(m[r]);
            }
        }
    }
    for (u32 rel = (u32)SUS_TILE + 1024u + threadIdx.x; rel < e_rel; rel += NT) {
        const u64 k = kt[rel];
        if (listed(rel, (u32)(k >> 32), hash0(k))) {
            const u32 n = atomicAdd(&s_nc, 1u);
            if (n < (u32)SUS_CAND) { s_cpos[n] = rel; s_cw[n] = (u32)(k >> 32); }
        }
    }
    __syncthreads();
    const u32 nc = s_nc;
    if (nc > (u32)SUS_CAND) {
        const i64 g0 = t0 + s_rel, g1 = t0 + e_rel - 1;
        for (i64 wd = (g0 >> 6) + threadIdx.x; wd <= (g1 >> 6); wd += NT) {
            u64 m = ~0ULL;
            if (wd == (g0 >> 6)) m &= ~0ULL << (g0 & 63);
            if (wd == (g1 >> 6)) m &= ~0ULL >> (63 - (g1 & 63));
            atomicOr(reinterpret_cast<ull *>(suspect64 + wd), (ull)m);
        }
        return;
    }
    const u32 nc4 = (nc + 3u) & ~3u, half = ((nc4 / 4 + 1) / 2) * 4;
    for (u32 a0 = 0; a0 < nc; a0 += NT / 2) {
        const u32 a = a0 + threadIdx.x / 2, part = threadIdx.x & 1u;
        const bool live = a < nc;
        const u32 wa = live ? s_cw[a] : 0u;
        u32 n_eq = 0, first = 0, last = 0;
        const u32 b0 = part ? half : 0u, b1 = part ? nc : (half < nc ? half : nc);
#pragma unroll 4
        for (u32 b = b0; b < b1; b += 4) {
            const u32x4 wl = *reinterpret_cast<const u32x4 *>(&s_cw[b]);
#pragma unroll
            for (u32 j = 0; j < 4; ++j)
                if (live && wl[j] == wa && b + j != a && b + j < b1) {
                    if (n_eq == 0) first = b + j;
                    last = b + j;
                    ++n_eq;
                }
        }
        {
            const u32 n_o = (u32)__shfl_xor((int)n_eq, 1), f_o = (u32)__shfl_xor((int)first, 1), l_o = (u32)__shfl_xor((int)last, 1);
            const u32 n_lo = part ? n_o : n_eq, f_lo = part ? f_o : first, l_lo = part ? l_o : last;
            const u32 n_hi = part ? n_eq : n_o, f_hi = part ? first : f_o, l_hi = part ? last : l_o;
            first = n_lo ? f_lo : f_hi;
            last = n_hi ? l_hi : l_lo;
            n_eq = n_lo + n_hi;
        }
        bool hit = n_eq > 2;
        if (n_eq >= 1 && n_eq <= 2 && part == 0) {
            const u64 ka = kt[s_cpos[a]], kb = kt[s_cpos[first]], kc = kt[s_cpos[last]];
            const u64 fa = L.full_key(hI, hO, ka);
            hit = (((ka ^ kb) >> F) == 0ULL && fa == L.full_key(hI, hO, kb)) || (((ka ^ kc) >> F) == 0ULL && fa == L.full_key(hI, hO, kc));
        }
        if (hit && part == 0) {
            const i64 p = t0 + s_cpos[a];
            atomicOr(reinterpret_cast<ull *>(suspect64 + (p >> 6)), 1ULL << (p & 63));
        }
    }
}
__global__ void k_popc_words64(const u64 *__restrict__ bits, i64 n_words, u32 *__restrict__ counts) {
    for (i64 w = (i64)blockIdx.x * blockDim.x + threadIdx.x; w < n_words; w += (i64)gridDim.x * blockDim.x) counts[w] = (u32)__popcll(bits[w]);
}
__global__ __launch_bounds__(256) void k_compact_suspects(const u64 *__restrict__ keys, const u64 *__restrict__ suspect64, const u32 *__restrict__ prefix,
                                                           i64 n_chunks, u64 *__restrict__ out) {
    const int lane = threadIdx.x & 63;
    for (i64 base = ((i64)blockIdx.x * 4 + (threadIdx.x >> 6)) * 16; base < n_chunks; base += (i64)gridDim.x * 64) {
        const i64 mine = base + (lane & 15);
        const u64 b = mine < n_chunks ? suspect64[mine] : 0ULL;
        u64 nz = __ballot(b != 0ULL) & 0xFFFFULL;
        while (nz) {
            const int l = __builtin_ctzll(nz);
            nz &= nz - 1;
            const u64 bb = __shfl(b, l);
            const i64 c = base + l;
            if ((bb >> lane) & 1ULL) out[(i64)prefix[c] + __popcll(bb & ((1ULL << lane) - 1ULL))] = keys ? keys[c * 64 + lane] : (u64)(c * 64 + lane);
        }
    }
}

static int pair_keys(const CleanupRun &r, bool bytes) {
    const PairOperands &p = r.rq.p;
    PairKeyArgs ka;
    ka.hI = r.hI.as<u64>(); ka.hO = r.hO_p; ka.keys = r.keys.as<u64>(); ka.bi = r.pl.L.bi; ka.bo = r.pl.L.bo; ka.o_base = 0; ka.squared = r.pl.squared ? 1 : 0;
    if (bytes) ka.ebytes = r.keys.as<unsigned char>();
    return mul_keys_dev(p.inner, p.Ni, p.outer, p.No, r.rq.W / 2, p.inner_is_left, ka);
}

static int mark_singles_packed(CleanupRun &r) {
    const CleanupPlan &pl = r.pl; const PairOperands &p = r.rq.p;
    const i64 Ni = p.Ni, No = p.No, Tk = pl.Tk; const double *ci = p.ci, *co = p.co; hipStream_t st = r.st;
    const i64 n_tiles = (Tk + SORT_TILE - 1) / SORT_TILE;
    SG_TRY(r.cfloor.alloc(16));
    const bool one_block = Ni <= 65536 && No <= 65536;
    if (!one_block) HIP_TRY(hipMemsetAsync(r.cfloor.p, 0xFF, 16, st));
    const bool two_ops = co != ci || No != Ni;
    if (one_block)
        hipLaunchKernelGGL(k_coeff_floor, dim3(1, two_ops ? 2 : 1), dim3(1024), 0, st, ci, Ni, co, No, r.cfloor.as<unsigned long long>(), 1);
    else {
        hipLaunchKernelGGL(k_coeff_floor, dim3(grid_for(Ni, 256, 256)), dim3(256), 0, st, ci, Ni, ci, Ni, r.cfloor.as<unsigned long long>(), 0);
        if (two_ops)
            hipLaunchKernelGGL(k_coeff_floor, dim3(grid_for(No, 256, 256)), dim3(256), 0, st, co, No, co, No, r.cfloor.as<unsigned long long>() + 1, 0);
    }
    const double *fl_i = r.cfloor.as<double>(), *fl_o = two_ops ? r.cfloor.as<double>() + 1 : r.cfloor.as<double>();
    if (r.sw.nofloor) fl_i = fl_o = nullptr;
    if (pl.key_bytes) {
        bump_counter(SYMGPU_CTR_FLOW_MARKED_FROM_BYTES);
        const i64 n_groups = (Tk + 63) / 64 * 4;
        hipLaunchKernelGGL(k_mark_bytes, dim3((unsigned)grid_for(n_groups, 256, 1 << 16)), dim3(256), 0, st, r.keys.as<u32x4>(), Tk, n_groups, Ni, ci, co,
                           pl.squared ? 1 : 0, r.rq.thr, r.rq.use_thr, r.markbits.as<unsigned short>(), r.e_lo.as<unsigned short>(), r.e_hi.as<unsigned short>(), fl_i, fl_o);
    } else {
        SG_TRY(r.sort_hist.alloc((size_t)n_tiles * 256 * sizeof(u32)));
        r.a.first_hist = r.sort_hist.as<u32>();
        hipLaunchKernelGGL(k_mark_singles<true>, dim3((unsigned)n_tiles), dim3(256), 0, st, r.keys.as<u64>(), (const double *)nullptr, Tk, pl.L, ci, co,
                           pl.squared ? 1 : 0, r.rq.thr, r.rq.use_thr, r.markbits.as<u64>(), r.e_lo.as<u64>(), r.e_hi.as<u64>(), r.a.first_hist, 64 - pl.nbits, n_tiles, fl_i, fl_o);
    }
    KERNEL_CHECK();
    return SYMGPU_OK;
}

int cleanup_hash_keys(CleanupRun &r) {
    const CleanupPlan &pl = r.pl; const CleanupRequest &rq = r.rq; const PairOperands &p = rq.p; hipStream_t st = r.st;
    if (!rq.pair) {
        SG_TRY(hash_rows_any(rq.rows, rq.T, rq.W, r.seed, r.keys.as<u64>(), r.idx.as<u32>()));
    } else {
        SG_TRY(hash_rows(p.inner, p.Ni, rq.W, r.hI.as<u64>()));
        if (!r.same_rows) SG_TRY(hash_rows(p.outer, p.No, rq.W, r.hO.as<u64>()));
        if (pl.packed) {
            SG_TRY(pair_keys(r, pl.key_bytes));
            if (pl.lazy) SG_TRY(mark_singles_packed(r));
        } else {
            if (!r.idx.p) {
                SG_TRY(r.idx.alloc((size_t)rq.T * 4));
                SG_TRY(r.idx2.alloc((size_t)rq.T * 4));
            }
            if (!r.pair_coeff.p) {
                SG_TRY(r.pair_coeff.alloc((size_t)rq.T * 16));
                SG_TRY(mul_coeff_dev(p.inner, p.ci, p.Ni, p.outer, p.co, 0, p.No, rq.W / 2, p.inner_is_left, r.pair_coeff.as<double>()));
                r.coeff = r.pair_coeff.as<double>();
            }
            hipLaunchKernelGGL(k_pair_keys, dim3(grid_for(rq.T)), dim3(256), 0, st, r.hI.as<u64>(), p.Ni, r.hO_p, rq.T, r.keys.as<u64>(), r.idx.as<u32>());
            KERNEL_CHECK();
        }
    }
    if (!pl.packed && pl.lazy) {
        hipLaunchKernelGGL(k_mark_singles<false>, dim3((unsigned)((rq.T + SORT_TILE - 1) / SORT_TILE)), dim3(256), 0, st, (const u64 *)nullptr, r.coeff, rq.T, pl.L, (const double *)nullptr,
                           (const double *)nullptr, 0, rq.thr, rq.use_thr, r.markbits.as<u64>(), (u64 *)nullptr, (u64 *)nullptr, (u32 *)nullptr, 0, (i64)0, (const double *)nullptr,
                           (const double *)nullptr);
        KERNEL_CHECK();
    }
    return SYMGPU_OK;
}

static int order_flagged(CleanupRun &r) {
    const CleanupPlan &pl = r.pl; const PairOperands &p = r.rq.p; CleanupRun::Attempt &a = r.a; hipStream_t st = r.st;
    const i64 Tk = pl.Tk;
    const int sus_pass = SUS_RUN_BITS / 8;
    const int lo = 64 - pl.nbits, hi = lo + 8 * sus_pass;
    const i64 n_sc = (Tk + 63) / 64;
    Scratch susbits, susprefix;
    SG_TRY(susbits.alloc((size_t)n_sc * 8 + 16));
    SG_TRY(susprefix.alloc((size_t)n_sc * 4));
    u32 *sustotal = susbits.as<u32>() + 2 * n_sc;
    SG_TRY(zero_two(susbits.p, (size_t)n_sc * 8 + 16, nullptr, 0));
    bool direct = false;
    SG_TRY(pair_dups_dev(r.hI.as<u64>(), p.Ni, r.hO_p, p.No, pl.squared, Tk, susbits.as<u64>(), sustotal + 1, &direct));
    u64 *part = r.keys.as<u64>(), *spare = r.keys2.as<u64>();
    bump_counter(direct ? SYMGPU_CTR_FLOW_FLAGS_HASH_TABLES : SYMGPU_CTR_FLOW_FLAGS_PARTIAL_SORT);
    if (!direct) {
        if (pl.key_bytes) SG_TRY(pair_keys(r, false));
        SortResult res;
        SG_TRY(radix_sort({part, spare, nullptr, nullptr, Tk, lo, hi, a.first_hist, SortForm::Launches}, &res));
        part = res.keys; spare = res.spare_keys;
        hipLaunchKernelGGL(k_find_suspects, dim3((unsigned)((Tk + SUS_TILE - 1) / SUS_TILE)), dim3(64 * SUS_WAVES), 0, st, part, Tk, pl.L, r.hI.as<u64>(),
                           r.hO_p, susbits.as<u64>(), sustotal + 1);
    }
    if (n_sc <= POPC_SCAN_SMALL_MAX) SG_TRY(popc_scan_small(susbits.as<u64>(), n_sc, -1, susprefix.as<u32>(), sustotal));
    else {
        hipLaunchKernelGGL(k_popc_words64, dim3(grid_for(n_sc)), dim3(256), 0, st, susbits.as<u64>(), n_sc, susprefix.as<u32>());
        KERNEL_CHECK();
        SG_TRY(exclusive_scan_u32(susprefix.as<u32>(), susprefix.as<u32>(), n_sc, sustotal));
    }
    u32 h_sus2[2] = {0, 0};
    {
        ReadBack rb;
        SG_TRY(read_back_post(sustotal, 2, nullptr, 0, &rb));
        const bool from_bytes = pl.key_bytes && direct;
        hipLaunchKernelGGL(k_compact_suspects, dim3((unsigned)grid_for((n_sc + 63) / 64, 1, 1 << 16)), dim3(256), 0, st, from_bytes ? (const u64 *)nullptr : part,
                           susbits.as<u64>(), susprefix.as<u32>(), n_sc, spare);
        if (from_bytes)
            hipLaunchKernelGGL(k_keys_of_indices, dim3(64), dim3(256), 0, st, spare, sustotal, r.keys.as<unsigned char>(), p.Ni, pl.squared ? 1 : 0, pl.L, r.hI.as<u64>(), r.hO_p);
        KERNEL_CHECK();
        SG_TRY(read_back_wait(&rb, h_sus2));
    }
    const u32 h_sus = h_sus2[0];
    if (h_sus2[1]) {
        bump_counter(SYMGPU_CTR_FLOW_FLAGS_GAVE_UP);
        for (u32 bit : PD_GIVEUP_BITS) if (direct && (h_sus2[1] & bit)) bump_counter(counter_of_giveup(bit));
    }
    if ((i64)h_sus * 16 > Tk || r.sw.suspects == 2 || h_sus2[1]) {
        bump_counter(SYMGPU_CTR_FLOW_SORTED_WHOLE);
        if (pl.key_bytes && direct) SG_TRY(pair_keys(r, false));
        SortResult res;
        SG_TRY(radix_sort({part, spare, nullptr, nullptr, Tk, direct ? lo : hi, 64, direct ? a.first_hist : nullptr, SortForm::Launches}, &res));
        a.ks = res.keys;
        return SYMGPU_OK;
    }
    bump_counter(SYMGPU_CTR_FLOW_SORTED_FLAGGED);
    a.sus_active = true;
    a.Tsort = h_sus;
    a.ks = part;
    if (a.Tsort == 0) return SYMGPU_OK;
    a.fix_bits = sorted_bits(a.Tsort, 64 - pl.L.F());
    const int sort_from = (!direct && 64 - a.fix_bits >= lo && 64 - a.fix_bits < hi) ? hi : 64 - a.fix_bits;
    SortResult res;
    SG_TRY(radix_sort({spare, part, nullptr, nullptr, a.Tsort, sort_from, 64, nullptr, SortForm::OneLaunchIfFits}, &res));
    a.sus_coop = res.one_launch;
    a.ks = res.keys;
    return SYMGPU_OK;
}

int cleanup_order(CleanupRun &r) {
    const CleanupPlan &pl = r.pl; CleanupRun::Attempt &a = r.a; const i64 Tk = pl.Tk;
    if (pl.sus_try) return order_flagged(r);
    if (pl.packed) bump_counter(SYMGPU_CTR_FLOW_COMPLETE_SORT);
    SortResult res;
    SG_TRY(radix_sort({r.keys.as<u64>(), r.keys2.as<u64>(), pl.packed ? nullptr : r.idx.as<u32>(), pl.packed ? nullptr : r.idx2.as<u32>(), Tk, 64 - pl.nbits, 64,
                       a.first_hist, SortForm::OneLaunchWherePays}, &res));
    a.sus_coop = res.one_launch;
    a.ks = res.keys;
    a.is = res.vals;
    return SYMGPU_OK;
}

}
```

symmer_amd/csrc/scan.hip:

```cpp
#include "sort.h"
#include "block_scan.h"
#include <stdlib.h>

namespace symgpu {

constexpr int SCAN_ITEMS = 8;
constexpr int SCAN_BLOCK = 256 * SCAN_ITEMS;

__global__ __launch_bounds__(256) void k_scan_block(const u32 *__restrict__ in, u32 *__restrict__ out, i64 n, u32 *__restrict__ block_sums) {
    __shared__ u32 s_wave[4];
    const i64 base = (i64)blockIdx.x * SCAN_BLOCK + (i64)threadIdx.x * SCAN_ITEMS;
    u32 v[SCAN_ITEMS];
    u32 sum = 0;
#pragma unroll
    for (int k = 0; k < SCAN_ITEMS; ++k) {
        v[k] = (base + k < n) ? in[base + k] : 0u;
        sum += v[k];
    }
    u32 total;
    u32 excl = block_excl_scan_256(sum, s_wave, &total);
#pragma unroll
    for (int k = 0; k < SCAN_ITEMS; ++k) {
        if (base + k < n) out[base + k] = excl;
        excl += v[k];
    }
    if (threadIdx.x == 0 && block_sums) block_sums[blockIdx.x] = total;
}

__global__ __launch_bounds__(256) void k_scan_add(u32 *__restrict__ out, i64 n, const u32 *__restrict__ block_offsets) {
    const i64 base = (i64)blockIdx.x * SCAN_BLOCK + (i64)threadIdx.x * SCAN_ITEMS;
    const u32 off = block_offsets[blockIdx.x];
#pragma unroll
    for (int k = 0; k < SCAN_ITEMS; ++k)
        if (base + k < n) out[base + k] += off;
}

__global__ void k_store_total(const u32 *__restrict__ last_in, const u32 *__restrict__ last_out, u32 *__restrict__ total) {
    *total = *last_in + *last_out;
}

constexpr int SCAN2_MAX_BLOCKS = 4096;
__global__ __launch_bounds__(256) void k_scan_sums(const u32 *__restrict__ in, i64 n, u32 *__restrict__ block_sums, u32 *__restrict__ total, u32 *__restrict__ ticket) {
    __shared__ u32 s_wave[4];
    __shared__ u32 s_last;
    const i64 base = (i64)blockIdx.x * SCAN_BLOCK + (i64)threadIdx.x * SCAN_ITEMS;
    u32 sum = 0;
#pragma unroll
    for (int k = 0; k < SCAN_ITEMS; ++k) sum += (base + k < n) ? in[base + k] : 0u;
    u32 tot;
    (void)block_excl_scan_256(sum, s_wave, &tot);
    if (threadIdx.x == 0) {
        __hip_atomic_store(block_sums + blockIdx.x, tot, __ATOMIC_RELAXED, __HIP_MEMORY_SCOPE_AGENT);
        asm volatile("s_waitcnt vmcnt(0)" ::: "memory");
        s_last = atomicAdd(ticket, 1u) == gridDim.x - 1 ? 1u : 0u;
    }
    __syncthreads();
    if (!s_last) return;
    constexpr int PER = SCAN2_MAX_BLOCKS / 256;
    u32 v[PER], mine = 0;
#pragma unroll
    for (int k = 0; k < PER; ++k) {
        const int b = threadIdx.x * PER + k;
        v[k] = b < (int)gridDim.x ? __hip_atomic_load(block_sums + b, __ATOMIC_RELAXED, __HIP_MEMORY_SCOPE_AGENT) : 0u;
        mine += v[k];
    }
    u32 all;
    u32 excl = block_excl_scan_256(mine, s_wave, &all);
#pragma unroll
    for (int k = 0; k < PER; ++k) {
        const int b = threadIdx.x * PER + k;
        if (b < (int)gridDim.x) block_sums[b] = excl;
        excl += v[k];
    }
    if (threadIdx.x == 0) { if (total) *total = all; *ticket = 0; }
}
__global__ __launch_bounds__(256) void k_scan_final(const u32 *__restrict__ in, u32 *__restrict__ out, i64 n, const u32 *__restrict__ block_offsets) {
    __shared__ u32 s_wave[4];
    const i64 base = (i64)blockIdx.x * SCAN_BLOCK + (i64)threadIdx.x * SCAN_ITEMS;
    const u32 off = block_offsets[blockIdx.x];
    u32 v[SCAN_ITEMS];
    u32 sum = 0;
#pragma unroll
    for (int k = 0; k < SCAN_ITEMS; ++k) {
        v[k] = (base + k < n) ? in[base + k] : 0u;
        sum += v[k];
    }
    u32 total;
    u32 excl = off + block_excl_scan_256(sum, s_wave, &total);
#pragma unroll
    for (int k = 0; k < SCAN_ITEMS; ++k) {
        if (base + k < n) out[base + k] = excl;
        excl += v[k];
    }
}

__global__ __launch_bounds__(1024) void k_popc_scan_small(const u64 *__restrict__ bits, i64 n, i64 n32, u32 *__restrict__ out, u32 *__restrict__ total) {
    __shared__ u32 s_wave[16];
    const int lane = threadIdx.x & 63, wave = threadIdx.x >> 6;
    const i64 b0 = (i64)threadIdx.x * 8;
    u32 cnt[8], sum = 0;
#pragma unroll
    for (int k = 0; k < 8; ++k) {
        const i64 w = b0 + k;
        u64 b = w < n ? bits[w] : 0ULL;
        if (n32 >= 0 && w == n - 1 && (n32 & 1)) b &= 0xFFFFFFFFULL;
        cnt[k] = (u32)__popcll(b);
        sum += cnt[k];
    }
    const u32 incl = wave_incl_scan(sum, lane);
    if (lane == 63) s_wave[wave] = incl;
    __syncthreads();
    u32 off = 0, tot = 0;
#pragma unroll
    for (int k = 0; k < 16; ++k) {
        const u32 sv = s_wave[k];
        if (k < wave) off += sv;
        tot += sv;
    }
    u32 run = off + incl - sum;
#pragma unroll
    for (int k = 0; k < 8; ++k) {
        if (b0 + k < n) out[b0 + k] = run;
        run += cnt[k];
    }
    if (threadIdx.x == 0 && total) *total = tot;
}
int popc_scan_small(const u64 *bits, i64 n, i64 n32, u32 *out, u32 *total_dev) {
    hipLaunchKernelGGL(k_popc_scan_small, dim3(1), dim3(1024), 0, ctx().stream, bits, n, n32, out, total_dev);
    KERNEL_CHECK();
    return SYMGPU_OK;
}

int exclusive_scan_u32(const u32 *in, u32 *out, i64 n, u32 *total_dev) {
    hipStream_t st = ctx().stream;
    if (n <= 0) {
        if (total_dev) HIP_TRY(hipMemsetAsync(total_dev, 0, sizeof(u32), st));
        return SYMGPU_OK;
    }
    const i64 nb = (n + SCAN_BLOCK - 1) / SCAN_BLOCK;
    const bool force_recursive = [] { const char *e = getenv("SYMGPU_SCAN_RECURSIVE"); return e && e[0] == '1'; }();
    if (nb <= SCAN2_MAX_BLOCKS && !force_recursive) {
        u32 *ticket;
        SG_TRY(sort_scan_ticket(&ticket));
        Scratch sums;
        SG_TRY(sums.alloc((size_t)nb * sizeof(u32)));
        hipLaunchKernelGGL(k_scan_sums, dim3((unsigned)nb), dim3(256), 0, st, in, n, sums.as<u32>(), total_dev, ticket + 1);
        hipLaunchKernelGGL(k_scan_final, dim3((unsigned)nb), dim3(256), 0, st, in, out, n, sums.as<u32>());
        KERNEL_CHECK();
        return SYMGPU_OK;
    }
    Scratch last;
    if (total_dev) {
        SG_TRY(last.alloc(sizeof(u32)));
        HIP_TRY(hipMemcpyAsync(last.p, in + (n - 1), sizeof(u32), hipMemcpyDeviceToDevice, st));
    }
    if (nb == 1) {
        hipLaunchKernelGGL(k_scan_block, dim3(1), dim3(256), 0, st, in, out, n, (u32 *)nullptr);
        KERNEL_CHECK();
    } else {
        Scratch sums;
        SG_TRY(sums.alloc((size_t)nb * sizeof(u32)));
        hipLaunchKernelGGL(k_scan_block, dim3((unsigned)nb), dim3(256), 0, st, in, out, n, sums.as<u32>());
        KERNEL_CHECK();
        SG_TRY(exclusive_scan_u32(sums.as<u32>(), sums.as<u32>(), nb, nullptr));
        hipLaunchKernelGGL(k_scan_add, dim3((unsigned)nb), dim3(256), 0, st, out, n, sums.as<u32>());
        KERNEL_CHECK();
    }
    if (total_dev) {
        hipLaunchKernelGGL(k_store_total, dim3(1), dim3(1), 0, st, last.as<u32>(), out + (n - 1), total_dev);
        KERNEL_CHECK();
    }
    return SYMGPU_OK;
}

__global__ __launch_bounds__(64) void k_ordered_sum(const f64x2 *__restrict__ v, i64 N, f64x2 *__restrict__ out) {
    __shared__ f64x2 s_p[2][64];
    const int lane = threadIdx.x;
    double re = 0.0, im = 0.0;
    int buf = 0;
    for (i64 base = 0; base < N; base += 64, buf ^= 1) {
        if (base + lane < N) s_p[buf][lane] = v[base + lane];
        __builtin_amdgcn_fence(__ATOMIC_RELEASE, "wavefront");
        __builtin_amdgcn_wave_barrier();
        __builtin_amdgcn_fence(__ATOMIC_ACQUIRE, "wavefront");
        if (lane == 0) {
            const int m = (int)(N - base < 64 ? N - base : 64);
            for (int k = 0; k < m; ++k) { const f64x2 p = s_p[buf][k]; re = __dadd_rn(re, p.x); im = __dadd_rn(im, p.y); }
        }
    }
    if (lane == 0) *out = f64x2{re, im};
}

int ordered_sum_dev(const f64x2 *v, i64 N, f64x2 *out) {
    hipLaunchKernelGGL(k_ordered_sum, dim3(1), dim3(64), 0, ctx().stream, v, N, out);
    KERNEL_CHECK();
    return SYMGPU_OK;
}

}
```

symmer_amd/csrc/sort.h:

```cpp
#pragma once
#include "common.h"

namespace symgpu {

int exclusive_scan_u32(const u32 *in, u32 *out, i64 n, u32 *total_dev );
constexpr i64 POPC_SCAN_SMALL_MAX = (i64)1 << 13;
int popc_scan_small(const u64 *bits, i64 n, i64 n32, u32 *out, u32 *total_dev);

constexpr int SORT_TILE = 4096;
constexpr int SORT_ONE_LAUNCH_MAX_TILES = 128;
constexpr int SORT_ONE_LAUNCH_TILES_KEYS = 48, SORT_ONE_LAUNCH_TILES_PAIRS = 32;
enum class SortForm {
    Launches,
    OneLaunchIfFits,
    OneLaunchWherePays,
};
struct SortRequest {
    u64 *keys, *keys_tmp;
    u32 *vals, *vals_tmp;
    i64 n;
    int begin_bit, end_bit;
    u32 *first_hist;
    SortForm want;
};
struct SortResult {
    u64 *keys, *spare_keys;
    u32 *vals, *spare_vals;
    bool one_launch;
};
bool sort_form(i64 n, bool has_vals, bool has_first_hist, SortForm want, bool one_launch_off);
int radix_sort(const SortRequest &rq, SortResult *res);

int sort_one_launch(const SortRequest &rq);
int sort_scan_ticket(u32 **ticket);
void sort_state_release(SortState &s);
int radix_sort_coop_check(bool *timed_out);
const u32 *radix_sort_coop_flag();
void radix_sort_coop_note(u32 flag, bool *timed_out);

}
```

symmer_amd/csrc/sort.hip:

```cpp
#include "sort.h"
#include "sort_tile.h"

namespace symgpu {

__global__ __launch_bounds__(256) void k_rs_hist(const u64 *__restrict__ keys, i64 n, int shift, i64 n_tiles, u32 *__restrict__ tile_hist) {
    __shared__ u32 h[256];
    h[threadIdx.x] = 0;
    __syncthreads();
    const i64 base = (i64)blockIdx.x * RS_TILE;
    u64 kk[RS_ITEMS];
#pragma unroll
    for (int k = 0; k < RS_ITEMS; ++k) {
        const i64 idx = base + k * 256 + threadIdx.x;
        kk[k] = idx < n ? keys[idx] : 0ULL;
    }
#pragma unroll
    for (int k = 0; k < RS_ITEMS; ++k)
        if (base + k * 256 + threadIdx.x < n) atomicAdd(&h[(kk[k] >> shift) & 255], 1u);
    __syncthreads();
    tile_hist[(i64)blockIdx.x * 256 + threadIdx.x] = h[threadIdx.x];
}

constexpr int RSC_MAX_CHUNKS = 128;
constexpr int RSC_MIN_LEN = 16;
__global__ __launch_bounds__(256) void k_rs_scan_cols(u32 *__restrict__ tile_hist, i64 n_tiles, i64 chunk_len, u32 *__restrict__ chunk_tot,
                                                       u32 *__restrict__ chunk_excl, u32 *__restrict__ row_total, u32 *__restrict__ ticket) {
    __shared__ u32 s_last;
    const int d = threadIdx.x;
    const i64 t0 = (i64)blockIdx.x * chunk_len, t1 = t0 + chunk_len < n_tiles ? t0 + chunk_len : n_tiles;
    u32 run = 0;
    for (i64 t = t0; t < t1; t += 16) {
        u32 v[16];
#pragma unroll
        for (int k = 0; k < 16; ++k) v[k] = t + k < t1 ? tile_hist[(t + k) * 256 + d] : 0u;
#pragma unroll
        for (int k = 0; k < 16; ++k) {
            if (t + k < t1) tile_hist[(t + k) * 256 + d] = run;
            run += v[k];
        }
    }
    __hip_atomic_store(chunk_tot + (i64)blockIdx.x * 256 + d, run, __ATOMIC_RELAXED, __HIP_MEMORY_SCOPE_AGENT);
    asm volatile("s_waitcnt vmcnt(0)" ::: "memory");
    __syncthreads();
    if (d == 0) s_last = atomicAdd(ticket, 1u) == gridDim.x - 1 ? 1u : 0u;
    __syncthreads();
    if (!s_last) return;
    u32 acc = 0;
    for (int c = 0; c < (int)gridDim.x; c += 32) {
        u32 v[32];
#pragma unroll
        for (int k = 0; k < 32; ++k)
            v[k] = c + k < (int)gridDim.x ? __hip_atomic_load(chunk_tot + (i64)(c + k) * 256 + d, __ATOMIC_RELAXED, __HIP_MEMORY_SCOPE_AGENT) : 0u;
#pragma unroll
        for (int k = 0; k < 32; ++k) {
            if (c + k < (int)gridDim.x) chunk_excl[(i64)(c + k) * 256 + d] = acc;
            acc += v[k];
        }
    }
    row_total[d] = acc;
    if (d == 0) *ticket = 0;
}

template <bool HAS_VALS>
__global__ __launch_bounds__(256) void k_rs_scatter(const u64 *__restrict__ keys, const u32 *__restrict__ vals, i64 n, int shift,
                                                     i64 n_tiles, const u32 *__restrict__ tile_off ,
                                                     const u32 *__restrict__ chunk_excl , i64 chunk_len,
                                                     const u32 *__restrict__ row_total ,
                                                     u64 *__restrict__ out_keys, u32 *__restrict__ out_vals) {
    __shared__ u64 s_key[RS_TILE];
    __shared__ u32 s_val[HAS_VALS ? RS_TILE : 1];
    __shared__ u32 s_cnt[4][256];
    __shared__ u32 s_dig_off[256];
    __shared__ u32 s_gbase[256];
    __shared__ u32 s_wave[4];

    const i64 per_xcd = (n_tiles + 7) / 8;
    const i64 tile = (i64)(blockIdx.x & 7) * per_xcd + (blockIdx.x >> 3);
    if (tile >= n_tiles) return;
    const i64 tile_base = tile * RS_TILE;
    const u32 goff = tile_off[tile * 256 + threadIdx.x] + chunk_excl[tile / chunk_len * 256 + threadIdx.x];
    const u32 gtot = row_total[threadIdx.x];
    u64 key[RS_ITEMS];
    u32 val[HAS_VALS ? RS_ITEMS : 1];
    u32 pos[RS_ITEMS];
    tile_load_items<TileMem::Plain, HAS_VALS>(keys, vals, tile_base, n, key, val);
    if (HAS_VALS) {
        asm volatile("" : "+v"(val[0]), "+v"(val[1]), "+v"(val[2]), "+v"(val[3]), "+v"(val[4]), "+v"(val[5]), "+v"(val[6]), "+v"(val[7]));
        asm volatile("" : "+v"(val[8]), "+v"(val[9]), "+v"(val[10]), "+v"(val[11]), "+v"(val[12]), "+v"(val[13]), "+v"(val[14]), "+v"(val[15]));
    }
#pragma unroll
    for (int k = 0; k < 4; ++k) s_cnt[k][threadIdx.x] = 0;
    {
        u32 all;
        s_gbase[threadIdx.x] = goff + block_excl_scan_256(gtot, s_wave, &all);
    }
    __syncthreads();
    tile_rank(key, shift, tile_base, n, s_cnt, pos);
    __syncthreads();
    (void)tile_digit_offsets(s_cnt, s_dig_off, s_wave);
    __syncthreads();
    tile_stage<HAS_VALS>(key, val, pos, shift, tile_base, n, s_dig_off, s_cnt, s_key, s_val);
    __syncthreads();
    tile_write_runs<TileMem::Plain, HAS_VALS>(s_key, s_val, shift, tile_base, n, s_dig_off, s_gbase, out_keys, out_vals);
}

bool sort_form(i64 n, bool has_vals, bool has_first_hist, SortForm want, bool one_launch_off) {
    if (want == SortForm::Launches || has_first_hist) return false;
    if (n <= 1) return true;
    const i64 n_tiles = (n + RS_TILE - 1) / RS_TILE;
    if (n_tiles > SORT_ONE_LAUNCH_MAX_TILES) return false;
    if (want == SortForm::OneLaunchWherePays && n_tiles > (has_vals ? SORT_ONE_LAUNCH_TILES_PAIRS : SORT_ONE_LAUNCH_TILES_KEYS)) return false;
    if (const char *e = SG_TUNE("SYMGPU_SORT_COOP")) if (e[0] == '0') return false;
    return !one_launch_off;
}

static_assert(RS_TILE == SORT_TILE, "the tile size callers form their first histogram with");
static int sort_launches(const SortRequest &rq) {
    const i64 n = rq.n;
    if (n >= ((i64)1 << 32)) {
        set_error("radix sort: n = %lld exceeds 2^32 - 1", (long long)n);
        return SYMGPU_E_INVALID;
    }
    hipStream_t st = ctx().stream;
    const i64 n_tiles = (n + RS_TILE - 1) / RS_TILE;
    u32 *ticket;
    SG_TRY(sort_scan_ticket(&ticket));
    const i64 chunk_len = (n_tiles + RSC_MAX_CHUNKS - 1) / RSC_MAX_CHUNKS > RSC_MIN_LEN ? (n_tiles + RSC_MAX_CHUNKS - 1) / RSC_MAX_CHUNKS : RSC_MIN_LEN;
    const unsigned n_chunks = (unsigned)((n_tiles + chunk_len - 1) / chunk_len);
    Scratch hist_own, scan;
    if (!rq.first_hist) SG_TRY(hist_own.alloc((size_t)n_tiles * 256 * sizeof(u32)));
    SG_TRY(scan.alloc((size_t)(1 + 2 * n_chunks) * 256 * sizeof(u32)));
    u32 *row_total = scan.as<u32>(), *chunk_tot = row_total + 256, *chunk_excl = chunk_tot + (size_t)n_chunks * 256;
    u32 *hist_p = rq.first_hist ? rq.first_hist : hist_own.as<u32>();
    u64 *ksrc = rq.keys, *kdst = rq.keys_tmp;
    u32 *vsrc = rq.vals, *vdst = rq.vals_tmp;
    for (int shift = rq.begin_bit; shift < rq.end_bit; shift += 8) {
        if (!(rq.first_hist && shift == rq.begin_bit)) {
            hipLaunchKernelGGL(k_rs_hist, dim3((unsigned)n_tiles), dim3(256), 0, st, ksrc, n, shift, n_tiles, hist_p);
            KERNEL_CHECK();
        }
        hipLaunchKernelGGL(k_rs_scan_cols, dim3(n_chunks), dim3(256), 0, st, hist_p, n_tiles, chunk_len, chunk_tot, chunk_excl, row_total, ticket);
        if (rq.vals)
            hipLaunchKernelGGL(k_rs_scatter<true>, dim3((unsigned)((n_tiles + 7) / 8 * 8)), dim3(256), 0, st, ksrc, vsrc, n, shift, n_tiles, hist_p, chunk_excl,
                               chunk_len, row_total, kdst, vdst);
        else
            hipLaunchKernelGGL(k_rs_scatter<false>, dim3((unsigned)((n_tiles + 7) / 8 * 8)), dim3(256), 0, st, ksrc, (const u32 *)nullptr, n, shift, n_tiles,
                               hist_p, chunk_excl, chunk_len, row_total, kdst, (u32 *)nullptr);
        KERNEL_CHECK();
        u64 *tk = ksrc; ksrc = kdst; kdst = tk;
        u32 *tv = vsrc; vsrc = vdst; vdst = tv;
    }
    return SYMGPU_OK;
}

int radix_sort(const SortRequest &rq, SortResult *res) {
    *res = SortResult{rq.keys, rq.keys_tmp, rq.vals, rq.vals_tmp, false};
    res->one_launch = sort_form(rq.n, rq.vals != nullptr, rq.first_hist != nullptr, rq.want, ctx().sort.coop_disabled);
    if (rq.n <= 1) return SYMGPU_OK;
    SG_TRY(res->one_launch ? sort_one_launch(rq) : sort_launches(rq));
    if (((rq.end_bit - rq.begin_bit + 7) / 8) & 1)
        *res = SortResult{rq.keys_tmp, rq.keys, rq.vals_tmp, rq.vals, res->one_launch};
    return SYMGPU_OK;
}

}

using namespace symgpu;

extern "C" {

int symgpu_debug_sort(uint64_t *keys, uint32_t *vals, int64_t n, int begin_bit, int end_bit, int form, int with_first_hist, int *form_ran) {
    SG_ENTER();
    SG_REQUIRE(form_ran && n >= 0 && (keys || n == 0), "debug_sort: null argument or negative n");
    SG_REQUIRE(begin_bit >= 0 && begin_bit < end_bit && end_bit <= 64 && (end_bit - begin_bit) % 8 == 0, "debug_sort: [begin_bit, end_bit) must be a multiple of 8 bits inside [0, 64)");
    SG_REQUIRE(form >= 0 && form <= 2, "debug_sort: form is 0 (a launch per step), 1 (one launch if it fits) or 2 (one launch where the library chooses it)");
    hipStream_t st = ctx().stream;
    Scratch keys_tmp, vals_tmp, hist;
    SG_TRY(keys_tmp.alloc((size_t)n * sizeof(u64)));
    if (vals) SG_TRY(vals_tmp.alloc((size_t)n * sizeof(u32)));
    u32 *first_hist = nullptr;
    if (with_first_hist) {
        const i64 n_tiles = (n + RS_TILE - 1) / RS_TILE;
        SG_TRY(hist.alloc((size_t)n_tiles * 256 * sizeof(u32)));
        first_hist = hist.as<u32>();
        if (n_tiles) hipLaunchKernelGGL(k_rs_hist, dim3((unsigned)n_tiles), dim3(256), 0, st, keys, n, begin_bit, n_tiles, first_hist);
        KERNEL_CHECK();
    }
    const SortForm want = form == 0 ? SortForm::Launches : form == 1 ? SortForm::OneLaunchIfFits : SortForm::OneLaunchWherePays;
    SortResult res;
    SG_TRY(radix_sort({keys, keys_tmp.as<u64>(), vals, vals_tmp.as<u32>(), n, begin_bit, end_bit, first_hist, want}, &res));
    if (res.keys != keys) {
        HIP_TRY(hipMemcpyAsync(keys, res.keys, (size_t)n * sizeof(u64), hipMemcpyDeviceToDevice, st));
        if (vals) HIP_TRY(hipMemcpyAsync(vals, res.vals, (size_t)n * sizeof(u32), hipMemcpyDeviceToDevice, st));
    }
    HIP_TRY(hipStreamSynchronize(st));
    *form_ran = res.one_launch ? 1 : 0;
    bool timed_out = false;
    if (res.one_launch) SG_TRY(radix_sort_coop_check(&timed_out));
    if (timed_out) { set_error("debug_sort: the one-launch sort gave up at a barrier; the buffers hold no sorted data"); return SYMGPU_E_HIP; }
    return SYMGPU_OK;
}

int symgpu_debug_scan(const uint32_t *in, uint32_t *out, int64_t n, uint32_t *total) {
    SG_ENTER();
    SG_REQUIRE(n >= 0 && ((in && out) || n == 0), "debug_scan: null argument or negative n");
    SG_TRY(exclusive_scan_u32(in, out, n, total));
    HIP_TRY(hipStreamSynchronize(ctx().stream));
    return SYMGPU_OK;
}

int symgpu_debug_popc_scan(const uint64_t *bits, int64_t n_words, int64_t n32, uint32_t *out, uint32_t *total) {
    SG_ENTER();
    SG_REQUIRE(bits && out && n_words >= 1 && n_words <= POPC_SCAN_SMALL_MAX, "debug_popc_scan: 1 to 8,192 words");
    SG_REQUIRE(n32 < 0 || n32 == 2 * n_words || n32 == 2 * n_words - 1, "debug_popc_scan: n32 is -1, 2 n_words or 2 n_words - 1");
    SG_TRY(popc_scan_small(bits, n_words, n32, out, total));
    HIP_TRY(hipStreamSynchronize(ctx().stream));
    return SYMGPU_OK;
}

}
```

symmer_amd/csrc/sort_coop.hip:

```cpp
#include "sort.h"
#include "sort_tile.h"

namespace symgpu {

typedef int32_t i32;

__device__ __forceinline__ bool coop_barrier(u32 *bar, u32 target, int G, u32 *s_flag) {
    asm volatile("s_waitcnt vmcnt(0)" ::: "memory");
    __syncthreads();
    if (G > 1 && threadIdx.x == 0) {
        atomicAdd(bar, 1u);
        u32 ok = 1;
        for (u32 spin = 0; (i32)(__hip_atomic_load(bar, __ATOMIC_RELAXED, __HIP_MEMORY_SCOPE_AGENT) - target) < 0; ++spin) {
            if (spin >= (1u << 22) || __hip_atomic_load(bar + 1, __ATOMIC_RELAXED, __HIP_MEMORY_SCOPE_AGENT) != 0) { ok = 0; break; }
            __builtin_amdgcn_s_sleep(1);
        }
        if (!ok) __hip_atomic_store(bar + 1, 1u, __ATOMIC_RELAXED, __HIP_MEMORY_SCOPE_AGENT);
        *s_flag = ok;
    }
    __syncthreads();
    return G == 1 || *s_flag != 0;
}

template <bool HAS_VALS>
__global__ __launch_bounds__(256) void k_rs_coop(u64 *__restrict__ buf_a, u64 *__restrict__ buf_b, u32 *__restrict__ val_a, u32 *__restrict__ val_b, i64 n, int begin_bit,
                                                  int n_passes, u32 *__restrict__ tile_hist , u32 *__restrict__ bar, u32 bar_base) {
    __shared__ u64 s_key[RS_TILE];
    __shared__ u32 s_val[HAS_VALS ? RS_TILE : 1];
    __shared__ u32 s_cnt[4][256];
    __shared__ u32 s_dig_off[256];
    __shared__ u32 s_gbase[256];
    __shared__ u32 s_wave[4];
    __shared__ u32 s_ok;
    const int G = gridDim.x, tile = blockIdx.x;
    const i64 tile_base = (i64)tile * RS_TILE;
    u32 n_bar = 0;
    for (int p = 0; p < n_passes; ++p) {
        const int shift = begin_bit + 8 * p;
        const u64 *src = (p & 1) ? buf_b : buf_a;
        u64 *dst = (p & 1) ? buf_a : buf_b;
        const u32 *vsrc = (p & 1) ? val_b : val_a;
        u32 *vdst = (p & 1) ? val_a : val_b;
#pragma unroll
        for (int k = 0; k < 4; ++k) s_cnt[k][threadIdx.x] = 0;
        __syncthreads();
        u64 key[RS_ITEMS];
        u32 pos[RS_ITEMS], val[HAS_VALS ? RS_ITEMS : 1];
        tile_load_items<TileMem::Agent, HAS_VALS>(src, vsrc, tile_base, n, key, val);
        tile_rank(key, shift, tile_base, n, s_cnt, pos);
        __syncthreads();
        const u32 my_count = tile_digit_offsets(s_cnt, s_dig_off, s_wave);
        __hip_atomic_store(&tile_hist[(i64)threadIdx.x * G + tile], my_count, __ATOMIC_RELAXED, __HIP_MEMORY_SCOPE_AGENT);
        if (!coop_barrier(bar, bar_base + (u32)G * (++n_bar), G, &s_ok)) return;
        {
            const int d = threadIdx.x;
            u32 all = 0, before = 0;
            if (G == 1) all = my_count;
            else
                for (int t0 = 0; t0 < G; t0 += 16) {
                    u32 x[16];
#pragma unroll
                    for (int k = 0; k < 16; ++k)
                        x[k] = t0 + k < G ? __hip_atomic_load(&tile_hist[(i64)d * G + t0 + k], __ATOMIC_RELAXED, __HIP_MEMORY_SCOPE_AGENT) : 0u;
                    asm volatile("" : "+v"(x[0]), "+v"(x[1]), "+v"(x[2]), "+v"(x[3]), "+v"(x[4]), "+v"(x[5]), "+v"(x[6]), "+v"(x[7]));
                    asm volatile("" : "+v"(x[8]), "+v"(x[9]), "+v"(x[10]), "+v"(x[11]), "+v"(x[12]), "+v"(x[13]), "+v"(x[14]), "+v"(x[15]));
#pragma unroll
                    for (int k = 0; k < 16; ++k) { all += x[k]; if (t0 + k < tile) before += x[k]; }
                }
            u32 total;
            s_gbase[d] = block_excl_scan_256(all, s_wave, &total) + before;
        }
        __syncthreads();
        tile_stage<HAS_VALS>(key, val, pos, shift, tile_base, n, s_dig_off, s_cnt, s_key, s_val);
        __syncthreads();
        tile_write_runs<TileMem::Agent, HAS_VALS>(s_key, s_val, shift, tile_base, n, s_dig_off, s_gbase, dst, vdst);
        if (!coop_barrier(bar, bar_base + (u32)G * (++n_bar), G, &s_ok)) return;
    }
}

int sort_one_launch(const SortRequest &rq) {
    Context &c = ctx();
    SortState &s = c.sort;
    hipStream_t st = c.stream;
    const i64 n_tiles = (rq.n + RS_TILE - 1) / RS_TILE;
    if (!s.coop_state) {
        HIP_TRY(hipMalloc((void **)&s.coop_state, (64 + 256 * SORT_ONE_LAUNCH_MAX_TILES) * sizeof(u32)));
        HIP_TRY(hipMemsetAsync(s.coop_state, 0, 64 * sizeof(u32), st));
        s.bar_base = 0;
    }
    const int n_passes = (rq.end_bit - rq.begin_bit + 7) / 8;
    const u32 arrivals = (u32)n_tiles * 2u * (u32)n_passes;
    if (s.bar_base > 0x70000000u - arrivals) {
        HIP_TRY(hipMemsetAsync(s.coop_state, 0, 64 * sizeof(u32), st));
        s.bar_base = 0;
    }
    if (rq.vals)
        hipLaunchKernelGGL((k_rs_coop<true>), dim3((unsigned)n_tiles), dim3(256), 0, st, rq.keys, rq.keys_tmp, rq.vals, rq.vals_tmp, rq.n, rq.begin_bit, n_passes, s.coop_state + 64,
                           s.coop_state, s.bar_base);
    else
        hipLaunchKernelGGL((k_rs_coop<false>), dim3((unsigned)n_tiles), dim3(256), 0, st, rq.keys, rq.keys_tmp, (u32 *)nullptr, (u32 *)nullptr, rq.n, rq.begin_bit, n_passes,
                           s.coop_state + 64, s.coop_state, s.bar_base);
    KERNEL_CHECK();
    s.bar_base += n_tiles > 1 ? arrivals : 0u;
    return SYMGPU_OK;
}

int sort_scan_ticket(u32 **ticket) {
    Context &c = ctx();
    if (!c.sort.scan_ticket) {
        HIP_TRY(hipMalloc((void **)&c.sort.scan_ticket, 256));
        HIP_TRY(hipMemsetAsync(c.sort.scan_ticket, 0, 256, c.stream));
    }
    *ticket = c.sort.scan_ticket;
    return SYMGPU_OK;
}
void sort_state_release(SortState &s) {
    if (s.coop_state) (void)hipFree(s.coop_state);
    if (s.scan_ticket) (void)hipFree(s.scan_ticket);
    s = SortState();
}

const u32 *radix_sort_coop_flag() {
    const SortState &s = ctx().sort;
    return (!s.coop_state || s.coop_disabled) ? nullptr : s.coop_state + 1;
}
void radix_sort_coop_note(u32 flag, bool *timed_out) {
    *timed_out = false;
    if (!flag) return;
    *timed_out = true;
    ctx().sort.coop_disabled = true;
    note_degraded("one-launch radix sort (k_rs_coop) off: an in-kernel barrier timed out (workgroups not co-resident?); sorts take one launch per pass");
}
int radix_sort_coop_check(bool *timed_out) {
    *timed_out = false;
    const u32 *p = radix_sort_coop_flag();
    if (!p) return SYMGPU_OK;
    u32 flag = 0;
    HIP_TRY(hipMemcpy(&flag, p, 4, hipMemcpyDeviceToHost));
    radix_sort_coop_note(flag, timed_out);
    return SYMGPU_OK;
}

}
```

Measured before the change: 25.70 billion.

## Add single-launch two-level popcount prefix and one-workgroup radix sort for cleanup tail

```diff
diff --git a/include/symgpu.h b/include/symgpu.h
--- a/include/symgpu.h
+++ b/include/symgpu.h
@@ -134,6 +134,7 @@
 int symgpu_debug_sort(uint64_t *keys, uint32_t *vals, int64_t n, int begin_bit, int end_bit, int form, int with_first_hist, int *form_ran);
 int symgpu_debug_scan(const uint32_t *in, uint32_t *out, int64_t n, uint32_t *total);
 int symgpu_debug_popc_scan(const uint64_t *bits, int64_t n_words, int64_t n32, uint32_t *out, uint32_t *total);
+int symgpu_debug_popc_prefix2(const uint64_t *bits, int64_t n_words, int64_t n32, uint32_t *local, uint32_t *group, uint32_t *total);
 int symgpu_degraded(char *buf, int len);
 int symgpu_debug_rotation_trace(uint64_t *out, int max_workgroups, int *n_workgroups);
 
diff --git a/symmer_amd/_lib.py b/symmer_amd/_lib.py
--- a/symmer_amd/_lib.py
+++ b/symmer_amd/_lib.py
@@ -41,6 +41,7 @@
     'symgpu_debug_sort': [P, P, c_i64, c_int, c_int, c_int, c_int, P],
     'symgpu_debug_scan': [P, P, c_i64, P],
     'symgpu_debug_popc_scan': [P, c_i64, c_i64, P, P],
+    'symgpu_debug_popc_prefix2': [P, c_i64, c_i64, P, P, P],
     'symgpu_debug_rotation_trace': [P, c_int, P],
     'symgpu_degraded': [P, c_int],
     'symgpu_membw_probe': [c_i64, P, P],
diff --git a/symmer_amd/csrc/cleanup.hip b/symmer_amd/csrc/cleanup.hip
--- a/symmer_amd/csrc/cleanup.hip
+++ b/symmer_amd/csrc/cleanup.hip
@@ -107,7 +107,7 @@
                                                      u32 Ni, int Wq, int wsh, const u32x4 *__restrict__ rows, const u32x4 *__restrict__ inner,
                                                      const u32x4 *__restrict__ outer, u32x4 *__restrict__ out_rows, double *__restrict__ out_coeff, LazyEmit lz,
                                                      u64 *__restrict__ out_first, int pfx_shift ,
-                                                     int interleaved) {
+                                                     int interleaved, const u32 *__restrict__ pfx_groups ) {
     __shared__ u32 s_i[4][64 * NW], s_o[4][64 * NW];
     const int lane = threadIdx.x & 63, wave = threadIdx.x >> 6;
     const i64 per_xcd = ((i64)gridDim.x + 7) / 8;
@@ -126,7 +126,7 @@
     }
     const u32 K = off[NW];
     if (K == 0) return;
-    const i64 p_base = wordprefix[w0 << pfx_shift];
+    const i64 p_base = (i64)wordprefix[w0 << pfx_shift] + (pfx_groups ? pfx_groups[w0 >> POPC_PREFIX2_SHIFT] : 0u);
     u32 o_min = 0xFFFFFFFFu, o_max = 0u;
     u32 ti_[NW], to_[NW], pw_[NW], el_[NW], eh_[NW];
     double2 ca_[NW], cb_[NW], cs_[NW];
@@ -244,12 +244,28 @@
         counts[w] = (u32)__popcll(b);
     }
 }
-int emit_prefix(const u32 *markbits_p, i64 T, Scratch &wordprefix, Scratch &total, bool wide) {
+int emit_prefix(const u32 *markbits_p, i64 T, EmitPrefix &pre, bool two_level, const LazyEmit *touch_lz) {
     hipStream_t st = ctx().stream;
+    Scratch &wordprefix = pre.wordprefix, &total = pre.total; const bool wide = pre.wide;
     const i64 n_words = (T + 31) / 32, n64 = (T + 63) / 64;
     const i64 n = wide ? n64 : n_words;
-    SG_TRY(wordprefix.alloc((size_t)n * 4));
+    two_level = two_level && wide && n64 > POPC_SCAN_SMALL_MAX;
+    SG_TRY(wordprefix.alloc((size_t)(n + (two_level ? popc_prefix2_groups(n64) : 0)) * 4));
     SG_TRY(total.alloc(32));
+    pre.groups = two_level ? wordprefix.as<u32>() + n : nullptr;
+    pre.touched = false;
+    if (two_level) {
+        const bool touch = touch_lz && T >= ((i64)1 << 23);
+        const u64 *maps[3] = {nullptr, nullptr, nullptr};
+        if (touch) {
+            maps[0] = touch_lz->mode ? reinterpret_cast<const u64 *>(touch_lz->patchbits) : nullptr;
+            maps[1] = touch_lz->mode == 1 ? reinterpret_cast<const u64 *>(touch_lz->e_lo) : nullptr;
+            maps[2] = touch_lz->mode == 1 ? reinterpret_cast<const u64 *>(touch_lz->e_hi) : nullptr;
+        }
+        pre.touched = touch_lz != nullptr;
+        return popc_prefix2(reinterpret_cast<const u64 *>(markbits_p), n64, n_words, wordprefix.as<u32>(), wordprefix.as<u32>() + n, total.as<u32>(), touch ? maps : nullptr,
+                            total.as<u32>() + 2);
+    }
     if (wide && n64 <= POPC_SCAN_SMALL_MAX) return popc_scan_small(reinterpret_cast<const u64 *>(markbits_p), n64, n_words, wordprefix.as<u32>(), total.as<u32>());
     if (wide) hipLaunchKernelGGL(k_popc_words64_tail, dim3(grid_for(n64)), dim3(256), 0, st, reinterpret_cast<const u64 *>(markbits_p), n64, n_words, wordprefix.as<u32>());
     else hipLaunchKernelGGL(k_popc_words, dim3(grid_for(n_words)), dim3(256), 0, st, markbits_p, n_words, wordprefix.as<u32>());
@@ -332,7 +348,7 @@
             SG_TRY(emit_order_begin(dst, (size_t)n_out * (size_t)(16 * Wq + 16), eo));
             ProfScope prof(3);
 #define LAUNCH_FUSED_S(P, TR, NWV, UV) hipLaunchKernelGGL((k_emit_fused<P, TR, NWV, UV>), gfu, dim3(256), 0, st, reinterpret_cast<const u64 *>(markbits_p), wordprefix.as<u32>(), T, sum_of_p, \
-                                               (u32)(pair ? Ni : 1), Wq, wsh, reinterpret_cast<const u32x4 *>(rows), pin, pout, dst, res->coeff, lz, res->first, pre.wide ? 0 : 1, eo.interleaved)
+                                               (u32)(pair ? Ni : 1), Wq, wsh, reinterpret_cast<const u32x4 *>(rows), pin, pout, dst, res->coeff, lz, res->first, pre.wide ? 0 : 1, eo.interleaved, pre.groups)
 #define LAUNCH_FUSED_U(P, TR, NWV) do { if (Us == 8) LAUNCH_FUSED_S(P, TR, NWV, 8); else if (Us == 2) LAUNCH_FUSED_S(P, TR, NWV, 2); else LAUNCH_FUSED_S(P, TR, NWV, 4); } while (0)
 #define LAUNCH_FUSED(P, TR) do { if (NWr == 1) LAUNCH_FUSED_U(P, TR, 1); else if (NWr == 4) LAUNCH_FUSED_U(P, TR, 4); else if (NWr == 8) LAUNCH_FUSED_U(P, TR, 8); \
                                  else LAUNCH_FUSED_U(P, TR, 2); } while (0)
diff --git a/symmer_amd/csrc/cleanup_common.h b/symmer_amd/csrc/cleanup_common.h
--- a/symmer_amd/csrc/cleanup_common.h
+++ b/symmer_amd/csrc/cleanup_common.h
@@ -43,6 +43,7 @@
     bool key_bytes = true;
     bool nofloor = false;
     bool emit_fused = true;
+    bool tail = true;
     i64 hs_waves = (i64)1 << 21;
     bool zero_seg = true;
     int emit_touch = -1;
@@ -81,7 +82,7 @@
     const u32 *patchbits = nullptr, *e_lo = nullptr, *e_hi = nullptr;
     const double *ci = nullptr, *co = nullptr, *coeff = nullptr;
 };
-struct EmitPrefix { Scratch wordprefix, total; i64 n_out = -1; bool touched = false, wide = false; };
+struct EmitPrefix { Scratch wordprefix, total; const u32 *groups = nullptr; i64 n_out = -1; bool touched = false, wide = false; };
 
 
 struct CleanupRun {
@@ -118,7 +119,7 @@
 int cleanup_diag_begin(CleanupRun &r);
 int cleanup_fixups(CleanupRun &r);
 int cleanup_segment_sums(CleanupRun &r);
-int emit_prefix(const u32 *markbits_p, i64 T, Scratch &wordprefix, Scratch &total, bool wide);
+int emit_prefix(const u32 *markbits_p, i64 T, EmitPrefix &pre, bool two_level, const LazyEmit *touch_lz = nullptr);
 int emit_touch(const u32 *markbits_p, i64 T, const LazyEmit &lz, EmitPrefix &pre);
 int cleanup_finish(u32 *markbits_p, const double *sum_of_p, i64 T, bool pair, const u64 *rows, int W, const u64 *inner, i64 Ni,
                    const u64 *outer, symgpu_op_t *out, int Wq_out, bool tri, const LazyEmit &lz, bool want_first, const CleanupSwitches &sw,
diff --git a/symmer_amd/csrc/cleanup_driver.hip b/symmer_amd/csrc/cleanup_driver.hip
--- a/symmer_amd/csrc/cleanup_driver.hip
+++ b/symmer_amd/csrc/cleanup_driver.hip
@@ -14,6 +14,7 @@
     if ((e = getenv("SYMGPU_CLEANUP_KEYBYTES"))) sw.key_bytes = e[0] != '0';
     sw.nofloor = getenv("SYMGPU_CLEANUP_NOFLOOR") != nullptr;
     if ((e = getenv("SYMGPU_EMIT_FUSED"))) sw.emit_fused = e[0] != '0';
+    if ((e = getenv("SYMGPU_CLEANUP_TAIL"))) sw.tail = e[0] != '0';
     if ((e = SG_TUNE("SYMGPU_HS_WAVES"))) sw.hs_waves = atoll(e);
     if ((e = SG_TUNE("SYMGPU_CLEANUP_ZEROSEG"))) sw.zero_seg = e[0] != '0';
     if ((e = SG_TUNE("SYMGPU_EMIT_TOUCH"))) sw.emit_touch = e[0] != '0';
@@ -53,9 +54,10 @@
 static int cleanup_status(CleanupRun &r, u32 hback[4]) {
     EmitPrefix &pre = r.pre;
     pre.wide = r.sw.fused(r.rq.W / 2);
-    SG_TRY(emit_prefix(r.markbits.as<u32>(), r.pl.Tk, pre.wordprefix, pre.total, pre.wide));
-    pre.touched = false;
-    if (pre.wide && r.sw.emit_touch == -1)
+    const LazyEmit lz = lazy_emit(r);
+    const bool touch_early = pre.wide && r.sw.emit_touch == -1;
+    SG_TRY(emit_prefix(r.markbits.as<u32>(), r.pl.Tk, pre, r.sw.tail, touch_early ? &lz : nullptr));
+    if (touch_early && !pre.touched)
         SG_TRY(emit_touch(r.markbits.as<u32>(), r.pl.Tk, lazy_emit(r), pre));
     SG_TRY(read_back_words(pre.total.as<u32>(), 1, r.collision.as<u32>(), 2, hback, r.a.sus_coop ? radix_sort_coop_flag() : nullptr));
     pre.n_out = hback[0];
diff --git a/symmer_amd/csrc/cleanup_keys.hip b/symmer_amd/csrc/cleanup_keys.hip
--- a/symmer_amd/csrc/cleanup_keys.hip
+++ b/symmer_amd/csrc/cleanup_keys.hip
@@ -417,7 +417,7 @@
     for (i64 w = (i64)blockIdx.x * blockDim.x + threadIdx.x; w < n_words; w += (i64)gridDim.x * blockDim.x) counts[w] = (u32)__popcll(bits[w]);
 }
 __global__ __launch_bounds__(256) void k_compact_suspects(const u64 *__restrict__ keys, const u64 *__restrict__ suspect64, const u32 *__restrict__ prefix,
-                                                           i64 n_chunks, u64 *__restrict__ out) {
+                                                           i64 n_chunks, u64 *__restrict__ out, const u32 *__restrict__ groups) {
     const int lane = threadIdx.x & 63;
     for (i64 base = ((i64)blockIdx.x * 4 + (threadIdx.x >> 6)) * 16; base < n_chunks; base += (i64)gridDim.x * 64) {
         const i64 mine = base + (lane & 15);
@@ -428,7 +428,8 @@
             nz &= nz - 1;
             const u64 bb = __shfl(b, l);
             const i64 c = base + l;
-            if ((bb >> lane) & 1ULL) out[(i64)prefix[c] + __popcll(bb & ((1ULL << lane) - 1ULL))] = keys ? keys[c * 64 + lane] : (u64)(c * 64 + lane);
+            if ((bb >> lane) & 1ULL)
+                out[(i64)prefix[c] + (groups ? groups[c >> POPC_PREFIX2_SHIFT] : 0u) + __popcll(bb & ((1ULL << lane) - 1ULL))] = keys ? keys[c * 64 + lane] : (u64)(c * 64 + lane);
         }
     }
 }
@@ -514,7 +515,7 @@
     const i64 n_sc = (Tk + 63) / 64;
     Scratch susbits, susprefix;
     SG_TRY(susbits.alloc((size_t)n_sc * 8 + 16));
-    SG_TRY(susprefix.alloc((size_t)n_sc * 4));
+    SG_TRY(susprefix.alloc((size_t)(n_sc + popc_prefix2_groups(n_sc)) * 4));
     u32 *sustotal = susbits.as<u32>() + 2 * n_sc;
     SG_TRY(zero_two(susbits.p, (size_t)n_sc * 8 + 16, nullptr, 0));
     bool direct = false;
@@ -529,8 +530,12 @@
         hipLaunchKernelGGL(k_find_suspects, dim3((unsigned)((Tk + SUS_TILE - 1) / SUS_TILE)), dim3(64 * SUS_WAVES), 0, st, part, Tk, pl.L, r.hI.as<u64>(),
                            r.hO_p, susbits.as<u64>(), sustotal + 1);
     }
+    const u32 *susgroups = nullptr;
     if (n_sc <= POPC_SCAN_SMALL_MAX) SG_TRY(popc_scan_small(susbits.as<u64>(), n_sc, -1, susprefix.as<u32>(), sustotal));
-    else {
+    else if (r.sw.tail) {
+        susgroups = susprefix.as<u32>() + n_sc;
+        SG_TRY(popc_prefix2(susbits.as<u64>(), n_sc, -1, susprefix.as<u32>(), susprefix.as<u32>() + n_sc, sustotal));
+    } else {
         hipLaunchKernelGGL(k_popc_words64, dim3(grid_for(n_sc)), dim3(256), 0, st, susbits.as<u64>(), n_sc, susprefix.as<u32>());
         KERNEL_CHECK();
         SG_TRY(exclusive_scan_u32(susprefix.as<u32>(), susprefix.as<u32>(), n_sc, sustotal));
@@ -541,7 +546,7 @@
         SG_TRY(read_back_post(sustotal, 2, nullptr, 0, &rb));
         const bool from_bytes = pl.key_bytes && direct;
         hipLaunchKernelGGL(k_compact_suspects, dim3((unsigned)grid_for((n_sc + 63) / 64, 1, 1 << 16)), dim3(256), 0, st, from_bytes ? (const u64 *)nullptr : part,
-                           susbits.as<u64>(), susprefix.as<u32>(), n_sc, spare);
+                           susbits.as<u64>(), susprefix.as<u32>(), n_sc, spare, susgroups);
         if (from_bytes)
             hipLaunchKernelGGL(k_keys_of_indices, dim3(64), dim3(256), 0, st, spare, sustotal, r.keys.as<unsigned char>(), p.Ni, pl.squared ? 1 : 0, pl.L, r.hI.as<u64>(), r.hO_p);
         KERNEL_CHECK();
@@ -568,7 +573,7 @@
     a.fix_bits = sorted_bits(a.Tsort, 64 - pl.L.F());
     const int sort_from = (!direct && 64 - a.fix_bits >= lo && 64 - a.fix_bits < hi) ? hi : 64 - a.fix_bits;
     SortResult res;
-    SG_TRY(radix_sort({spare, part, nullptr, nullptr, a.Tsort, sort_from, 64, nullptr, SortForm::OneLaunchIfFits}, &res));
+    SG_TRY(radix_sort({spare, part, nullptr, nullptr, a.Tsort, sort_from, 64, nullptr, r.sw.tail ? SortForm::OneWorkgroupIfFits : SortForm::OneLaunchIfFits}, &res));
     a.sus_coop = res.one_launch;
     a.ks = res.keys;
     return SYMGPU_OK;
diff --git a/symmer_amd/csrc/scan.hip b/symmer_amd/csrc/scan.hip
--- a/symmer_amd/csrc/scan.hip
+++ b/symmer_amd/csrc/scan.hip
@@ -127,6 +127,76 @@
 }
 int popc_scan_small(const u64 *bits, i64 n, i64 n32, u32 *out, u32 *total_dev) {
     hipLaunchKernelGGL(k_popc_scan_small, dim3(1), dim3(1024), 0, ctx().stream, bits, n, n32, out, total_dev);
+    KERNEL_CHECK();
+    return SYMGPU_OK;
+}
+
+struct PopcTouch { const u64 *map[3]; };
+__global__ __launch_bounds__(256) void k_popc_prefix2(const u64 *__restrict__ bits, i64 n, i64 n32, u32 *__restrict__ local, u32 *__restrict__ group,
+                                                       u32 *__restrict__ total, u32 *__restrict__ ticket, PopcTouch touch, u32 *__restrict__ sink) {
+    __shared__ u32 s_wave[4];
+    __shared__ u32 s_last;
+    constexpr int PER = POPC_PREFIX2_GROUP / 256;
+    const i64 b0 = (i64)blockIdx.x * POPC_PREFIX2_GROUP + (i64)threadIdx.x * PER;
+    u32 cnt[PER], sum = 0;
+#pragma unroll
+    for (int k = 0; k < PER; ++k) {
+        const i64 w = b0 + k;
+        u64 b = w < n ? bits[w] : 0ULL;
+        if (n32 >= 0 && w == n - 1 && (n32 & 1)) b &= 0xFFFFFFFFULL;
+        cnt[k] = (u32)__popcll(b);
+        sum += cnt[k];
+    }
+    u64 acc = ~0ULL;
+#pragma unroll
+    for (int m = 0; m < 3; ++m)
+        if (touch.map[m]) {
+#pragma unroll
+            for (int k = 0; k < PER; ++k) if (b0 + k < n) acc &= touch.map[m][b0 + k];
+        }
+    if (sink && acc == 0xDEADBEEFDEADBEEFULL) *sink = 1u;
+    u32 tot;
+    u32 run = block_excl_scan_256(sum, s_wave, &tot);
+#pragma unroll
+    for (int k = 0; k < PER; ++k) {
+        if (b0 + k < n) local[b0 + k] = run;
+        run += cnt[k];
+    }
+    if (threadIdx.x == 0) {
+        __hip_atomic_store(group + blockIdx.x, tot, __ATOMIC_RELAXED, __HIP_MEMORY_SCOPE_AGENT);
+        asm volatile("s_waitcnt vmcnt(0)" ::: "memory");
+        s_last = atomicAdd(ticket, 1u) == gridDim.x - 1 ? 1u : 0u;
+    }
+    __syncthreads();
+    if (!s_last) return;
+    u32 carry = 0;
+    for (u32 g0 = 0; g0 < gridDim.x; g0 += 256 * 8) {
+        u32 v[8], mine = 0;
+#pragma unroll
+        for (int k = 0; k < 8; ++k) {
+            const u32 g = g0 + threadIdx.x * 8 + k;
+            v[k] = g < gridDim.x ? __hip_atomic_load(group + g, __ATOMIC_RELAXED, __HIP_MEMORY_SCOPE_AGENT) : 0u;
+            mine += v[k];
+        }
+        u32 all;
+        u32 excl = carry + block_excl_scan_256(mine, s_wave, &all);
+#pragma unroll
+        for (int k = 0; k < 8; ++k) {
+            const u32 g = g0 + threadIdx.x * 8 + k;
+            if (g < gridDim.x) group[g] = excl;
+            excl += v[k];
+        }
+        carry += all;
+    }
+    if (threadIdx.x == 0) { if (total) *total = carry; *ticket = 0; }
+}
+int popc_prefix2(const u64 *bits, i64 n, i64 n32, u32 *local, u32 *group, u32 *total_dev, const u64 *const *touch, u32 *sink) {
+    u32 *ticket;
+    SG_TRY(sort_scan_ticket(&ticket));
+    PopcTouch pt{{nullptr, nullptr, nullptr}};
+    for (int m = 0; m < 3 && touch; ++m) pt.map[m] = touch[m];
+    hipLaunchKernelGGL(k_popc_prefix2, dim3((unsigned)popc_prefix2_groups(n)), dim3(256), 0, ctx().stream, bits, n, n32, local, group, total_dev, ticket + 2, pt,
+                       touch ? sink : (u32 *)nullptr);
     KERNEL_CHECK();
     return SYMGPU_OK;
 }
diff --git a/symmer_amd/csrc/sort.h b/symmer_amd/csrc/sort.h
--- a/symmer_amd/csrc/sort.h
+++ b/symmer_amd/csrc/sort.h
@@ -6,15 +6,21 @@
 int exclusive_scan_u32(const u32 *in, u32 *out, i64 n, u32 *total_dev );
 constexpr i64 POPC_SCAN_SMALL_MAX = (i64)1 << 13;
 int popc_scan_small(const u64 *bits, i64 n, i64 n32, u32 *out, u32 *total_dev);
+constexpr int POPC_PREFIX2_SHIFT = 10, POPC_PREFIX2_GROUP = 1 << POPC_PREFIX2_SHIFT;
+inline i64 popc_prefix2_groups(i64 n) { return (n + POPC_PREFIX2_GROUP - 1) >> POPC_PREFIX2_SHIFT; }
+int popc_prefix2(const u64 *bits, i64 n, i64 n32, u32 *local, u32 *group, u32 *total_dev, const u64 *const *touch = nullptr, u32 *sink = nullptr);
 
 constexpr int SORT_TILE = 4096;
 constexpr int SORT_ONE_LAUNCH_MAX_TILES = 128;
 constexpr int SORT_ONE_LAUNCH_TILES_KEYS = 48, SORT_ONE_LAUNCH_TILES_PAIRS = 32;
+constexpr i64 SORT_ONE_WORKGROUP_MAX = 16384;
 enum class SortForm {
     Launches,
     OneLaunchIfFits,
     OneLaunchWherePays,
+    OneWorkgroupIfFits,
 };
+enum class SortRuns { Launches, OneLaunch, OneWorkgroup };
 struct SortRequest {
     u64 *keys, *keys_tmp;
     u32 *vals, *vals_tmp;
@@ -27,11 +33,13 @@
     u64 *keys, *spare_keys;
     u32 *vals, *spare_vals;
     bool one_launch;
+    bool one_workgroup;
 };
-bool sort_form(i64 n, bool has_vals, bool has_first_hist, SortForm want, bool one_launch_off);
+SortRuns sort_form(i64 n, bool has_vals, bool has_first_hist, SortForm want, bool one_launch_off);
 int radix_sort(const SortRequest &rq, SortResult *res);
 
 int sort_one_launch(const SortRequest &rq);
+int sort_one_workgroup(const SortRequest &rq);
 int sort_scan_ticket(u32 **ticket);
 void sort_state_release(SortState &s);
 int radix_sort_coop_check(bool *timed_out);
diff --git a/symmer_amd/csrc/sort.hip b/symmer_amd/csrc/sort.hip
--- a/symmer_amd/csrc/sort.hip
+++ b/symmer_amd/csrc/sort.hip
@@ -104,14 +104,18 @@
     tile_write_runs<TileMem::Plain, HAS_VALS>(s_key, s_val, shift, tile_base, n, s_dig_off, s_gbase, out_keys, out_vals);
 }
 
-bool sort_form(i64 n, bool has_vals, bool has_first_hist, SortForm want, bool one_launch_off) {
-    if (want == SortForm::Launches || has_first_hist) return false;
-    if (n <= 1) return true;
+SortRuns sort_form(i64 n, bool has_vals, bool has_first_hist, SortForm want, bool one_launch_off) {
+    if (want == SortForm::Launches || has_first_hist) return SortRuns::Launches;
+    if (want == SortForm::OneWorkgroupIfFits) {
+        if (!has_vals && n <= SORT_ONE_WORKGROUP_MAX) return SortRuns::OneWorkgroup;
+        want = SortForm::OneLaunchIfFits;
+    }
+    if (n <= 1) return SortRuns::OneLaunch;
     const i64 n_tiles = (n + RS_TILE - 1) / RS_TILE;
-    if (n_tiles > SORT_ONE_LAUNCH_MAX_TILES) return false;
-    if (want == SortForm::OneLaunchWherePays && n_tiles > (has_vals ? SORT_ONE_LAUNCH_TILES_PAIRS : SORT_ONE_LAUNCH_TILES_KEYS)) return false;
-    if (const char *e = SG_TUNE("SYMGPU_SORT_COOP")) if (e[0] == '0') return false;
-    return !one_launch_off;
+    if (n_tiles > SORT_ONE_LAUNCH_MAX_TILES) return SortRuns::Launches;
+    if (want == SortForm::OneLaunchWherePays && n_tiles > (has_vals ? SORT_ONE_LAUNCH_TILES_PAIRS : SORT_ONE_LAUNCH_TILES_KEYS)) return SortRuns::Launches;
+    if (const char *e = SG_TUNE("SYMGPU_SORT_COOP")) if (e[0] == '0') return SortRuns::Launches;
+    return one_launch_off ? SortRuns::Launches : SortRuns::OneLaunch;
 }
 
 static_assert(RS_TILE == SORT_TILE, "the tile size callers form their first histogram with");
@@ -154,12 +158,12 @@
 }
 
 int radix_sort(const SortRequest &rq, SortResult *res) {
-    *res = SortResult{rq.keys, rq.keys_tmp, rq.vals, rq.vals_tmp, false};
-    res->one_launch = sort_form(rq.n, rq.vals != nullptr, rq.first_hist != nullptr, rq.want, ctx().sort.coop_disabled);
+    const SortRuns runs = sort_form(rq.n, rq.vals != nullptr, rq.first_hist != nullptr, rq.want, ctx().sort.coop_disabled);
+    *res = SortResult{rq.keys, rq.keys_tmp, rq.vals, rq.vals_tmp, runs == SortRuns::OneLaunch, runs == SortRuns::OneWorkgroup};
     if (rq.n <= 1) return SYMGPU_OK;
-    SG_TRY(res->one_launch ? sort_one_launch(rq) : sort_launches(rq));
+    SG_TRY(runs == SortRuns::OneWorkgroup ? sort_one_workgroup(rq) : runs == SortRuns::OneLaunch ? sort_one_launch(rq) : sort_launches(rq));
     if (((rq.end_bit - rq.begin_bit + 7) / 8) & 1)
-        *res = SortResult{rq.keys_tmp, rq.keys, rq.vals_tmp, rq.vals, res->one_launch};
+        *res = SortResult{rq.keys_tmp, rq.keys, rq.vals_tmp, rq.vals, res->one_launch, res->one_workgroup};
     return SYMGPU_OK;
 }
 
@@ -173,7 +177,7 @@
     SG_ENTER();
     SG_REQUIRE(form_ran && n >= 0 && (keys || n == 0), "debug_sort: null argument or negative n");
     SG_REQUIRE(begin_bit >= 0 && begin_bit < end_bit && end_bit <= 64 && (end_bit - begin_bit) % 8 == 0, "debug_sort: [begin_bit, end_bit) must be a multiple of 8 bits inside [0, 64)");
-    SG_REQUIRE(form >= 0 && form <= 2, "debug_sort: form is 0 (a launch per step), 1 (one launch if it fits) or 2 (one launch where the library chooses it)");
+    SG_REQUIRE(form >= 0 && form <= 3, "debug_sort: form is 0 (a launch per step), 1 (one launch if it fits), 2 (one launch where the library chooses it) or 3 (one workgroup if it fits)");
     hipStream_t st = ctx().stream;
     Scratch keys_tmp, vals_tmp, hist;
     SG_TRY(keys_tmp.alloc((size_t)n * sizeof(u64)));
@@ -186,7 +190,7 @@
         if (n_tiles) hipLaunchKernelGGL(k_rs_hist, dim3((unsigned)n_tiles), dim3(256), 0, st, keys, n, begin_bit, n_tiles, first_hist);
         KERNEL_CHECK();
     }
-    const SortForm want = form == 0 ? SortForm::Launches : form == 1 ? SortForm::OneLaunchIfFits : SortForm::OneLaunchWherePays;
+    const SortForm want = form == 0 ? SortForm::Launches : form == 1 ? SortForm::OneLaunchIfFits : form == 2 ? SortForm::OneLaunchWherePays : SortForm::OneWorkgroupIfFits;
     SortResult res;
     SG_TRY(radix_sort({keys, keys_tmp.as<u64>(), vals, vals_tmp.as<u32>(), n, begin_bit, end_bit, first_hist, want}, &res));
     if (res.keys != keys) {
@@ -194,7 +198,7 @@
         if (vals) HIP_TRY(hipMemcpyAsync(vals, res.vals, (size_t)n * sizeof(u32), hipMemcpyDeviceToDevice, st));
     }
     HIP_TRY(hipStreamSynchronize(st));
-    *form_ran = res.one_launch ? 1 : 0;
+    *form_ran = res.one_workgroup ? 2 : res.one_launch ? 1 : 0;
     bool timed_out = false;
     if (res.one_launch) SG_TRY(radix_sort_coop_check(&timed_out));
     if (timed_out) { set_error("debug_sort: the one-launch sort gave up at a barrier; the buffers hold no sorted data"); return SYMGPU_E_HIP; }
@@ -218,4 +222,13 @@
     return SYMGPU_OK;
 }
 
-}
+int symgpu_debug_popc_prefix2(const uint64_t *bits, int64_t n_words, int64_t n32, uint32_t *local, uint32_t *group, uint32_t *total) {
+    SG_ENTER();
+    SG_REQUIRE(bits && local && group && n_words >= 1 && n_words < ((int64_t)1 << 31), "debug_popc_prefix2: null argument or n_words outside 1 .. 2^31 - 1");
+    SG_REQUIRE(n32 < 0 || n32 == 2 * n_words || n32 == 2 * n_words - 1, "debug_popc_prefix2: n32 is -1, 2 n_words or 2 n_words - 1");
+    SG_TRY(popc_prefix2(bits, n_words, n32, local, group, total));
+    HIP_TRY(hipStreamSynchronize(ctx().stream));
+    return SYMGPU_OK;
+}
+
+}
diff --git a/symmer_amd/csrc/sort_coop.hip b/symmer_amd/csrc/sort_coop.hip
--- a/symmer_amd/csrc/sort_coop.hip
+++ b/symmer_amd/csrc/sort_coop.hip
@@ -105,6 +105,94 @@
     return SYMGPU_OK;
 }
 
+constexpr int OWG_WAVES = 16, OWG_THREADS = 64 * OWG_WAVES;
+static_assert((i64)OWG_WAVES * RS_WSEG == SORT_ONE_WORKGROUP_MAX, "sixteen keys per lane");
+__global__ __launch_bounds__(OWG_THREADS) void k_rs_one_workgroup(const u64 *src, u64 *dst , i64 n, int begin_bit, int n_passes) {
+    __shared__ u64 s_key[SORT_ONE_WORKGROUP_MAX];
+    __shared__ u32 s_cnt[OWG_WAVES][256];
+    __shared__ u32 s_dig_off[256];
+    __shared__ u32 s_wave[OWG_WAVES];
+    const int lane = threadIdx.x & 63, wave = threadIdx.x >> 6;
+    const u64 lt_mask = (1ULL << lane) - 1ULL;
+    u64 key[RS_ITEMS];
+    u32 pos[RS_ITEMS];
+#pragma unroll
+    for (int r = 0; r < RS_ITEMS; ++r) {
+        const i64 idx = (i64)wave * RS_WSEG + r * 64 + lane;
+        key[r] = idx < n ? src[idx] : ~0ULL;
+    }
+    for (int p = 0; p < n_passes; ++p) {
+        const int shift = begin_bit + 8 * p;
+#pragma unroll
+        for (int k = 0; k < 256 / 64; ++k) s_cnt[wave][k * 64 + lane] = 0;
+        __builtin_amdgcn_fence(__ATOMIC_ACQ_REL, "wavefront");
+        __builtin_amdgcn_wave_barrier();
+#pragma unroll
+        for (int r = 0; r < RS_ITEMS; ++r) {
+            if ((i64)wave * RS_WSEG + r * 64 >= n) break;
+            const bool valid = (i64)wave * RS_WSEG + r * 64 + lane < n;
+            const u32 d = (u32)(key[r] >> shift) & 255u;
+            const u64 m = match_digit(d, valid);
+            const u32 rank = __popcll(m & lt_mask);
+            const u32 count = __popcll(m);
+            u32 base = 0;
+            if (valid) base = s_cnt[wave][d];
+            __builtin_amdgcn_fence(__ATOMIC_ACQ_REL, "wavefront");
+            __builtin_amdgcn_wave_barrier();
+            if (valid && rank == 0) s_cnt[wave][d] = base + count;
+            __builtin_amdgcn_fence(__ATOMIC_ACQ_REL, "wavefront");
+            __builtin_amdgcn_wave_barrier();
+            pos[r] = base + rank;
+        }
+        __syncthreads();
+        {
+            u32 run = 0;
+            if (threadIdx.x < 256) {
+#pragma unroll
+                for (int k = 0; k < OWG_WAVES; ++k) {
+                    const u32 c = s_cnt[k][threadIdx.x];
+                    s_cnt[k][threadIdx.x] = run;
+                    run += c;
+                }
+            }
+            const u32 incl = wave_incl_scan(run, lane);
+            if (lane == 63) s_wave[wave] = incl;
+            __syncthreads();
+            u32 off = 0;
+#pragma unroll
+            for (int k = 0; k < 4; ++k) if (k < wave) off += s_wave[k];
+            if (threadIdx.x < 256) s_dig_off[threadIdx.x] = off + incl - run;
+        }
+        __syncthreads();
+        const bool last = p == n_passes - 1;
+#pragma unroll
+        for (int r = 0; r < RS_ITEMS; ++r) {
+            if ((i64)wave * RS_WSEG + r * 64 + lane < n) {
+                const u32 d = (u32)(key[r] >> shift) & 255u;
+                const u32 slot = s_dig_off[d] + s_cnt[wave][d] + pos[r];
+                if (last) dst[slot] = key[r];
+                else s_key[slot] = key[r];
+            }
+        }
+        if (last) break;
+        __syncthreads();
+#pragma unroll
+        for (int r = 0; r < RS_ITEMS; ++r) {
+            const i64 idx = (i64)wave * RS_WSEG + r * 64 + lane;
+            key[r] = idx < n ? s_key[idx] : ~0ULL;
+        }
+        __syncthreads();
+    }
+}
+int sort_one_workgroup(const SortRequest &rq) {
+    const int n_passes = (rq.end_bit - rq.begin_bit + 7) / 8;
+    if (rq.n > SORT_ONE_WORKGROUP_MAX || rq.vals) { set_error("radix sort: the one-workgroup form takes up to %lld bare keys", (long long)SORT_ONE_WORKGROUP_MAX); return SYMGPU_E_INVALID; }
+    if (n_passes <= 0) return SYMGPU_OK;
+    hipLaunchKernelGGL(k_rs_one_workgroup, dim3(1), dim3(OWG_THREADS), 0, ctx().stream, rq.keys, (n_passes & 1) ? rq.keys_tmp : rq.keys, rq.n, rq.begin_bit, n_passes);
+    KERNEL_CHECK();
+    return SYMGPU_OK;
+}
+
 int sort_scan_ticket(u32 **ticket) {
     Context &c = ctx();
     if (!c.sort.scan_ticket) {
```

Result: no change. 25.72 billion (median of 2 runs) (+0.1%).
